# AnyLoc/AnyLoc

Hardware: NVIDIA H100
Metric: images/sec end-to-end DINOv2-VLAD descriptors (higher is better)
Workload: dtype f32-equivalent (tensor-core fp16 3-term split, fp32 accumulate)

## Files before the change

anyloc_b200/csrc/attention_tc.cu:

```cuda
#include <stdlib.h>
#include "common.cuh"

namespace anyloc {
namespace atc {

constexpr int BQ = 64, BKV = 64, HD = 64, WARPS = 4, THREADS = WARPS * 32;

template <bool F16, bool BF16 = false> struct Cfg {
  using T = typename std::conditional<BF16, __nv_bfloat16, typename std::conditional<F16, __half, float>::type>::type;
  static constexpr int PITCH = F16 ? HD + 8 : HD + 4;
  static constexpr int MAT = BKV * PITCH;
  static constexpr int NMAT = BF16 ? 2 : 4;
  static constexpr int STAGE = NMAT * MAT;
  static constexpr int SMEM_BYTES = 2 * STAGE * (int)sizeof(T);
  static constexpr int CHUNKS_PER_ROW = HD * (int)sizeof(T) / 16;
};

__device__ __forceinline__ void cp_async16(uint32_t dst, const void* src, bool valid) {
  asm volatile("cp.async.cg.shared.global [%0], [%1], 16, %2;" ::"r"(dst), "l"(src), "r"(valid ? 16 : 0) : "memory");
}
__device__ __forceinline__ void cp_async_commit() { asm volatile("cp.async.commit_group;" ::: "memory"); }
template <int N>
__device__ __forceinline__ void cp_async_wait() { asm volatile("cp.async.wait_group %0;" ::"n"(N) : "memory"); }

__device__ __forceinline__ void mma_f16(float* d, const uint32_t* a, uint32_t b0, uint32_t b1) {
  asm volatile(
      "mma.sync.aligned.m16n8k16.row.col.f32.f16.f16.f32 {%0, %1, %2, %3}, {%4, %5, %6, %7}, {%8, %9}, "
      "{%0, %1, %2, %3};"
      : "+f"(d[0]), "+f"(d[1]), "+f"(d[2]), "+f"(d[3])
      : "r"(a[0]), "r"(a[1]), "r"(a[2]), "r"(a[3]), "r"(b0), "r"(b1));
}
__device__ __forceinline__ void mma_bf16(float* d, const uint32_t* a, uint32_t b0, uint32_t b1) {
  asm volatile(
      "mma.sync.aligned.m16n8k16.row.col.f32.bf16.bf16.f32 {%0, %1, %2, %3}, {%4, %5, %6, %7}, {%8, %9}, "
      "{%0, %1, %2, %3};"
      : "+f"(d[0]), "+f"(d[1]), "+f"(d[2]), "+f"(d[3])
      : "r"(a[0]), "r"(a[1]), "r"(a[2]), "r"(a[3]), "r"(b0), "r"(b1));
}
__device__ __forceinline__ void mma_tf32(float* d, const uint32_t* a, uint32_t b0, uint32_t b1) {
  asm volatile(
      "mma.sync.aligned.m16n8k8.row.col.f32.tf32.tf32.f32 {%0, %1, %2, %3}, {%4, %5, %6, %7}, {%8, %9}, "
      "{%0, %1, %2, %3};"
      : "+f"(d[0]), "+f"(d[1]), "+f"(d[2]), "+f"(d[3])
      : "r"(a[0]), "r"(a[1]), "r"(a[2]), "r"(a[3]), "r"(b0), "r"(b1));
}
__device__ __forceinline__ void ldsm_x4(uint32_t addr, uint32_t* r) {
  asm volatile("ldmatrix.sync.aligned.m8n8.x4.shared.b16 {%0, %1, %2, %3}, [%4];"
               : "=r"(r[0]), "=r"(r[1]), "=r"(r[2]), "=r"(r[3]) : "r"(addr));
}
__device__ __forceinline__ void ldsm_x4_t(uint32_t addr, uint32_t* r) {
  asm volatile("ldmatrix.sync.aligned.m8n8.x4.trans.shared.b16 {%0, %1, %2, %3}, [%4];"
               : "=r"(r[0]), "=r"(r[1]), "=r"(r[2]), "=r"(r[3]) : "r"(addr));
}
__device__ __forceinline__ float ex2(float x) {
  float y; asm("ex2.approx.ftz.f32 %0, %1;" : "=f"(y) : "f"(x)); return y;
}
__device__ __forceinline__ uint32_t f2u(float x) { return __float_as_uint(x); }
template <typename E>
__device__ __forceinline__ uint32_t ld_h2(const E* p) { return *reinterpret_cast<const uint32_t*>(p); }

template <bool F16, bool VARLEN, bool BF16 = false>
__device__ __forceinline__ void attention_cta(const void* __restrict__ qkv_hi_, const void* __restrict__ qkv_lo_, int T,
                                              int D, void* __restrict__ o_hi_, void* __restrict__ o_lo_,
                                              const VarlenAttnTable* tab) {
  static_assert(!BF16 || F16, "bf16 uses the 2-byte (k16) layout");
  using C = Cfg<F16, BF16>;
  using E = typename C::T;
  extern __shared__ __align__(16) uint8_t smem_raw[];
  E* smem = reinterpret_cast<E*>(smem_raw);
  const E* qkv_hi = reinterpret_cast<const E*>(qkv_hi_);
  const E* qkv_lo = reinterpret_cast<const E*>(qkv_lo_);
  int qt = blockIdx.x;
  const int h = blockIdx.y, b = blockIdx.z;
  const int warp = threadIdx.x >> 5, lane = threadIdx.x & 31, g = lane >> 2, t4 = lane & 3;
  const size_t ld = 3 * (size_t)D;
  size_t img0 = (size_t)b * T;
  if constexpr (VARLEN) {
    int lo = 0, hi = tab->n - 1;
    while (lo < hi) {
      const int mid = (lo + hi + 1) >> 1;
      if (tab->tile0[mid] <= qt) lo = mid; else hi = mid - 1;
    }
    qt -= tab->tile0[lo]; T = tab->len[lo]; img0 = (size_t)tab->row0[lo];
  }
  const int nblk = (T + BKV - 1) / BKV;
  constexpr bool SCALED = F16 && !BF16;
  const float P_SCALE = SCALED ? 1024.0f : 1.0f;
  const float kScale = 0.125f * 1.4426950408889634f * (SCALED ? 1.0f / (kActScale * kActScale) : 1.0f);

  auto load_block = [&](int j, int buf) {
    E* st = smem + buf * C::STAGE;
    constexpr int PIECES = C::NMAT * BKV * C::CHUNKS_PER_ROW;
    for (int p = threadIdx.x; p < PIECES; p += THREADS) {
      const int mat = p / (BKV * C::CHUNKS_PER_ROW), r = (p / C::CHUNKS_PER_ROW) % BKV, c = p % C::CHUNKS_PER_ROW;
      const int key = j * BKV + r;
      const bool valid = key < T;
      const E* src = (!BF16 && (mat & 1)) ? qkv_lo : qkv_hi;
      const bool is_k = BF16 ? mat == 0 : mat < 2;
      const size_t col = (size_t)(is_k ? D : 2 * D) + (size_t)h * HD + (size_t)c * (16 / sizeof(E));
      const E* gp = src + (valid ? (img0 + key) * ld + col : 0);
      cp_async16((uint32_t)__cvta_generic_to_shared(st + mat * C::MAT + r * C::PITCH + c * (16 / sizeof(E))), gp, valid);
    }
    cp_async_commit();
  };
  load_block(0, 0);

  const int q0 = qt * BQ + warp * 16 + g, q1 = q0 + 8;
  constexpr int QK_STEPS = F16 ? HD / 16 : HD / 8;
  uint32_t qa_hi[QK_STEPS][4], qa_lo[QK_STEPS][4];
  {
    const size_t r0 = (img0 + q0) * ld + (size_t)h * HD, r1 = (img0 + q1) * ld + (size_t)h * HD;
    const bool v0 = q0 < T, v1 = q1 < T;
#pragma unroll
    for (int ks = 0; ks < QK_STEPS; ++ks) {
      if constexpr (F16) {
        const int c0 = ks * 16 + 2 * t4, c1 = c0 + 8;
        qa_hi[ks][0] = v0 ? ld_h2(qkv_hi + r0 + c0) : 0u; qa_hi[ks][1] = v1 ? ld_h2(qkv_hi + r1 + c0) : 0u;
        qa_hi[ks][2] = v0 ? ld_h2(qkv_hi + r0 + c1) : 0u; qa_hi[ks][3] = v1 ? ld_h2(qkv_hi + r1 + c1) : 0u;
        if (BF16) continue;
        qa_lo[ks][0] = v0 ? ld_h2(qkv_lo + r0 + c0) : 0u; qa_lo[ks][1] = v1 ? ld_h2(qkv_lo + r1 + c0) : 0u;
        qa_lo[ks][2] = v0 ? ld_h2(qkv_lo + r0 + c1) : 0u; qa_lo[ks][3] = v1 ? ld_h2(qkv_lo + r1 + c1) : 0u;
      } else {
        const int c0 = ks * 8 + t4, c1 = c0 + 4;
        qa_hi[ks][0] = v0 ? f2u(qkv_hi[r0 + c0]) : 0u; qa_hi[ks][1] = v1 ? f2u(qkv_hi[r1 + c0]) : 0u;
        qa_hi[ks][2] = v0 ? f2u(qkv_hi[r0 + c1]) : 0u; qa_hi[ks][3] = v1 ? f2u(qkv_hi[r1 + c1]) : 0u;
        qa_lo[ks][0] = v0 ? f2u(qkv_lo[r0 + c0]) : 0u; qa_lo[ks][1] = v1 ? f2u(qkv_lo[r1 + c0]) : 0u;
        qa_lo[ks][2] = v0 ? f2u(qkv_lo[r0 + c1]) : 0u; qa_lo[ks][3] = v1 ? f2u(qkv_lo[r1 + c1]) : 0u;
      }
    }
  }

  float o[8][4];
  float m0 = -INFINITY, m1 = -INFINITY, l0 = 0.f, l1 = 0.f;
#pragma unroll
  for (int nd = 0; nd < 8; ++nd) o[nd][0] = o[nd][1] = o[nd][2] = o[nd][3] = 0.f;

  for (int j = 0; j < nblk; ++j) {
    const int buf = j & 1;
    if (j + 1 < nblk) { load_block(j + 1, buf ^ 1); cp_async_wait<1>(); }
    else cp_async_wait<0>();
    __syncthreads();
    const E* sK_hi = smem + buf * C::STAGE;
    const E* sK_lo = sK_hi + C::MAT;
    const E* sV_hi = sK_hi + (BF16 ? 1 : 2) * C::MAT;
    const E* sV_lo = sK_hi + 3 * C::MAT;

    float s[8][4];
#pragma unroll
    for (int nt = 0; nt < 8; ++nt) s[nt][0] = s[nt][1] = s[nt][2] = s[nt][3] = 0.f;
#pragma unroll
    for (int nt = 0; nt < 8; ++nt) {
      if constexpr (F16) {
        const int key = nt * 8 + (lane & 7), dim = 8 * (lane >> 3);
#pragma unroll
        for (int c = 0; c < 2; ++c) {
          uint32_t bh[4], bl[4];
          ldsm_x4((uint32_t)__cvta_generic_to_shared(sK_hi + key * C::PITCH + 32 * c + dim), bh);
          if constexpr (BF16) {
#pragma unroll
            for (int u = 0; u < 2; ++u) mma_bf16(s[nt], qa_hi[2 * c + u], bh[2 * u], bh[2 * u + 1]);
            continue;
          }
          ldsm_x4((uint32_t)__cvta_generic_to_shared(sK_lo + key * C::PITCH + 32 * c + dim), bl);
#pragma unroll
          for (int u = 0; u < 2; ++u) {
            const int ks = 2 * c + u;
            mma_f16(s[nt], qa_hi[ks], bh[2 * u], bh[2 * u + 1]);
            mma_f16(s[nt], qa_lo[ks], bh[2 * u], bh[2 * u + 1]);
            mma_f16(s[nt], qa_hi[ks], bl[2 * u], bl[2 * u + 1]);
          }
        }
      } else {
        const float* kh = sK_hi + (nt * 8 + g) * C::PITCH;
        const float* kl = sK_lo + (nt * 8 + g) * C::PITCH;
#pragma unroll
        for (int ks = 0; ks < QK_STEPS; ++ks) {
          const uint32_t bh0 = f2u(kh[ks * 8 + t4]), bh1 = f2u(kh[ks * 8 + t4 + 4]);
          const uint32_t bl0 = f2u(kl[ks * 8 + t4]), bl1 = f2u(kl[ks * 8 + t4 + 4]);
          mma_tf32(s[nt], qa_hi[ks], bh0, bh1);
          mma_tf32(s[nt], qa_lo[ks], bh0, bh1);
          mma_tf32(s[nt], qa_hi[ks], bl0, bl1);
        }
      }
    }

    float mx0 = m0, mx1 = m1;
#pragma unroll
    for (int nt = 0; nt < 8; ++nt) {
      const int key = j * BKV + nt * 8 + 2 * t4;
#pragma unroll
      for (int e = 0; e < 2; ++e) {
        const bool live = key + e < T;
        s[nt][e] = live ? s[nt][e] * kScale : -INFINITY;
        s[nt][2 + e] = live ? s[nt][2 + e] * kScale : -INFINITY;
        mx0 = fmaxf(mx0, s[nt][e]); mx1 = fmaxf(mx1, s[nt][2 + e]);
      }
    }
    mx0 = fmaxf(mx0, __shfl_xor_sync(0xffffffffu, mx0, 1)); mx0 = fmaxf(mx0, __shfl_xor_sync(0xffffffffu, mx0, 2));
    mx1 = fmaxf(mx1, __shfl_xor_sync(0xffffffffu, mx1, 1)); mx1 = fmaxf(mx1, __shfl_xor_sync(0xffffffffu, mx1, 2));
    const float alpha0 = ex2(m0 - mx0), alpha1 = ex2(m1 - mx1);
    m0 = mx0; m1 = mx1;
    float r0 = 0.f, r1 = 0.f;
#pragma unroll
    for (int nt = 0; nt < 8; ++nt) {
      s[nt][0] = ex2(s[nt][0] - mx0); s[nt][1] = ex2(s[nt][1] - mx0);
      s[nt][2] = ex2(s[nt][2] - mx1); s[nt][3] = ex2(s[nt][3] - mx1);
      r0 += s[nt][0] + s[nt][1]; r1 += s[nt][2] + s[nt][3];
    }
    l0 = l0 * alpha0 + r0; l1 = l1 * alpha1 + r1;

    float pv[8][4];
#pragma unroll
    for (int nd = 0; nd < 8; ++nd) pv[nd][0] = pv[nd][1] = pv[nd][2] = pv[nd][3] = 0.f;
    if constexpr (BF16) {
#pragma unroll
      for (int ks = 0; ks < 4; ++ks) {
        uint32_t ph[4];
        ph[0] = pack_bf16x2(s[2 * ks][0], s[2 * ks][1]);
        ph[1] = pack_bf16x2(s[2 * ks][2], s[2 * ks][3]);
        ph[2] = pack_bf16x2(s[2 * ks + 1][0], s[2 * ks + 1][1]);
        ph[3] = pack_bf16x2(s[2 * ks + 1][2], s[2 * ks + 1][3]);
        const int key = ks * 16 + (lane & 7) + 8 * ((lane >> 3) & 1), dsel = 8 * (lane >> 4);
#pragma unroll
        for (int nd = 0; nd < 8; nd += 2) {
          uint32_t vh[4];
          ldsm_x4_t((uint32_t)__cvta_generic_to_shared(sV_hi + key * C::PITCH + nd * 8 + dsel), vh);
#pragma unroll
          for (int u = 0; u < 2; ++u) mma_bf16(pv[nd + u], ph, vh[2 * u], vh[2 * u + 1]);
        }
      }
    } else if constexpr (F16) {
#pragma unroll
      for (int ks = 0; ks < 4; ++ks) {
        uint32_t ph[4], pl[4];
        split_f16x2(s[2 * ks][0] * P_SCALE, s[2 * ks][1] * P_SCALE, ph[0], pl[0]);
        split_f16x2(s[2 * ks][2] * P_SCALE, s[2 * ks][3] * P_SCALE, ph[1], pl[1]);
        split_f16x2(s[2 * ks + 1][0] * P_SCALE, s[2 * ks + 1][1] * P_SCALE, ph[2], pl[2]);
        split_f16x2(s[2 * ks + 1][2] * P_SCALE, s[2 * ks + 1][3] * P_SCALE, ph[3], pl[3]);
        const int key = ks * 16 + (lane & 7) + 8 * ((lane >> 3) & 1), dsel = 8 * (lane >> 4);
#pragma unroll
        for (int nd = 0; nd < 8; nd += 2) {
          uint32_t vh[4], vl[4];
          ldsm_x4_t((uint32_t)__cvta_generic_to_shared(sV_hi + key * C::PITCH + nd * 8 + dsel), vh);
          ldsm_x4_t((uint32_t)__cvta_generic_to_shared(sV_lo + key * C::PITCH + nd * 8 + dsel), vl);
#pragma unroll
          for (int u = 0; u < 2; ++u) {
            mma_f16(pv[nd + u], ph, vh[2 * u], vh[2 * u + 1]);
            mma_f16(pv[nd + u], pl, vh[2 * u], vh[2 * u + 1]);
            mma_f16(pv[nd + u], ph, vl[2 * u], vl[2 * u + 1]);
          }
        }
      }
    } else {
#pragma unroll
      for (int ks = 0; ks < 8; ++ks) {
        uint32_t ph[4], pl[4];
        float hh, ll;
        split_tf32(s[ks][0], hh, ll); ph[0] = f2u(hh); pl[0] = f2u(ll);
        split_tf32(s[ks][2], hh, ll); ph[1] = f2u(hh); pl[1] = f2u(ll);
        split_tf32(s[ks][1], hh, ll); ph[2] = f2u(hh); pl[2] = f2u(ll);
        split_tf32(s[ks][3], hh, ll); ph[3] = f2u(hh); pl[3] = f2u(ll);
        const float* vh0 = sV_hi + (ks * 8 + 2 * t4) * C::PITCH;
        const float* vl0 = sV_lo + (ks * 8 + 2 * t4) * C::PITCH;
#pragma unroll
        for (int nd = 0; nd < 8; ++nd) {
          const uint32_t bh0 = f2u(vh0[nd * 8 + g]), bh1 = f2u(vh0[C::PITCH + nd * 8 + g]);
          const uint32_t bl0 = f2u(vl0[nd * 8 + g]), bl1 = f2u(vl0[C::PITCH + nd * 8 + g]);
          mma_tf32(pv[nd], ph, bh0, bh1);
          mma_tf32(pv[nd], pl, bh0, bh1);
          mma_tf32(pv[nd], ph, bl0, bl1);
        }
      }
    }
#pragma unroll
    for (int nd = 0; nd < 8; ++nd) {
      o[nd][0] = o[nd][0] * alpha0 + pv[nd][0]; o[nd][1] = o[nd][1] * alpha0 + pv[nd][1];
      o[nd][2] = o[nd][2] * alpha1 + pv[nd][2]; o[nd][3] = o[nd][3] * alpha1 + pv[nd][3];
    }
    __syncthreads();
  }

  l0 += __shfl_xor_sync(0xffffffffu, l0, 1); l0 += __shfl_xor_sync(0xffffffffu, l0, 2);
  l1 += __shfl_xor_sync(0xffffffffu, l1, 1); l1 += __shfl_xor_sync(0xffffffffu, l1, 2);
  const float inv0 = 1.0f / (l0 * P_SCALE), inv1 = 1.0f / (l1 * P_SCALE);
#pragma unroll
  for (int half = 0; half < 2; ++half) {
    const int q = half ? q1 : q0;
    if (q >= T) continue;
    const float inv = half ? inv1 : inv0;
    const size_t off = (img0 + q) * (size_t)D + (size_t)h * HD + 2 * t4;
#pragma unroll
    for (int nd = 0; nd < 8; ++nd) {
      const float a = o[nd][2 * half] * inv, c = o[nd][2 * half + 1] * inv;
      if constexpr (BF16) {
        *reinterpret_cast<uint32_t*>(reinterpret_cast<__nv_bfloat16*>(o_hi_) + off + nd * 8) = pack_bf16x2(a, c);
      } else if constexpr (F16) {
        uint32_t hh, ll;
        split_f16x2(a, c, hh, ll);
        *reinterpret_cast<uint32_t*>(reinterpret_cast<__half*>(o_hi_) + off + nd * 8) = hh;
        *reinterpret_cast<uint32_t*>(reinterpret_cast<__half*>(o_lo_) + off + nd * 8) = ll;
      } else {
        float2 hh, ll;
        split_tf32(a, hh.x, ll.x); split_tf32(c, hh.y, ll.y);
        *reinterpret_cast<float2*>(reinterpret_cast<float*>(o_hi_) + off + nd * 8) = hh;
        *reinterpret_cast<float2*>(reinterpret_cast<float*>(o_lo_) + off + nd * 8) = ll;
      }
    }
  }
}

template <bool F16, bool BF16 = false>
__global__ void __launch_bounds__(THREADS)
attention_tc_kernel(const void* __restrict__ qkv_hi_, const void* __restrict__ qkv_lo_, int T, int D,
                    void* __restrict__ o_hi_, void* __restrict__ o_lo_) {
  attention_cta<F16, false, BF16>(qkv_hi_, qkv_lo_, T, D, o_hi_, o_lo_, nullptr);
}

template <bool F16, bool BF16 = false>
__global__ void __launch_bounds__(THREADS)
attention_tc_varlen_kernel(const void* __restrict__ qkv_hi_, const void* __restrict__ qkv_lo_,
                           const __grid_constant__ VarlenAttnTable tab, int D, void* __restrict__ o_hi_,
                           void* __restrict__ o_lo_) {
  attention_cta<F16, true, BF16>(qkv_hi_, qkv_lo_, 0, D, o_hi_, o_lo_, &tab);
}

__global__ void __launch_bounds__(256)
qkv_to_f16_kernel(const float* __restrict__ qkv_hi, const float* __restrict__ qkv_lo, size_t n, __half* __restrict__ q16_hi,
                  __half* __restrict__ q16_lo) {
  for (size_t i = blockIdx.x * (size_t)blockDim.x + threadIdx.x; i < n; i += (size_t)gridDim.x * blockDim.x) {
    __half hh, ll; split_f16((qkv_hi[i] + qkv_lo[i]) * kActScale, hh, ll);
    q16_hi[i] = hh; q16_lo[i] = ll;
  }
}

}

int attention_tc_launch(const void* qkv_hi, const void* qkv_lo, int B, int T, int D, int heads, void* o_hi, void* o_lo,
                        int fmt, cudaStream_t st) {
  using namespace atc;
  ANYLOC_REQUIRE(D == heads * HD, "attention_tc: head_dim must be 64 (D=%d heads=%d)", D, heads);
  ANYLOC_REQUIRE(B <= 65535 && heads <= 65535, "attention_tc: grid too large (B=%d heads=%d)", B, heads);
  static unsigned long long attr_seen = 0;
  if (first_use_on_this_device(&attr_seen)) {
    ANYLOC_CHECK_CUDA(cudaFuncSetAttribute(attention_tc_kernel<true>, cudaFuncAttributeMaxDynamicSharedMemorySize,
                                           Cfg<true>::SMEM_BYTES));
    ANYLOC_CHECK_CUDA(cudaFuncSetAttribute(attention_tc_kernel<false>, cudaFuncAttributeMaxDynamicSharedMemorySize,
                                           Cfg<false>::SMEM_BYTES));
  }
  const dim3 grid(cdiv(T, BQ), heads, B);
  if (fmt == ANYLOC_PAIR_BF16)
    attention_tc_kernel<true, true><<<grid, THREADS, Cfg<true, true>::SMEM_BYTES, st>>>(qkv_hi, qkv_lo, T, D, o_hi, o_lo);
  else if (fmt == ANYLOC_PAIR_F16) attention_tc_kernel<true><<<grid, THREADS, Cfg<true>::SMEM_BYTES, st>>>(qkv_hi, qkv_lo, T, D, o_hi, o_lo);
  else attention_tc_kernel<false><<<grid, THREADS, Cfg<false>::SMEM_BYTES, st>>>(qkv_hi, qkv_lo, T, D, o_hi, o_lo);
  ANYLOC_CHECK_LAUNCH();
  return ANYLOC_OK;
}

int attention_tc_varlen_launch(const void* qkv_hi, const void* qkv_lo, const VarlenAttnTable& tab, int n_tiles, int D,
                               int heads, void* o_hi, void* o_lo, int fmt, cudaStream_t st) {
  using namespace atc;
  ANYLOC_REQUIRE(D == heads * HD, "attention_tc: head_dim must be 64 (D=%d heads=%d)", D, heads);
  ANYLOC_REQUIRE(heads <= 65535, "attention_tc: grid too large (heads=%d)", heads);
  static unsigned long long attr_seen = 0;
  if (first_use_on_this_device(&attr_seen)) {
    ANYLOC_CHECK_CUDA(cudaFuncSetAttribute(attention_tc_varlen_kernel<true>,
                                           cudaFuncAttributeMaxDynamicSharedMemorySize, Cfg<true>::SMEM_BYTES));
    ANYLOC_CHECK_CUDA(cudaFuncSetAttribute(attention_tc_varlen_kernel<false>,
                                           cudaFuncAttributeMaxDynamicSharedMemorySize, Cfg<false>::SMEM_BYTES));
  }
  const dim3 grid(n_tiles, heads);
  if (fmt == ANYLOC_PAIR_BF16)
    attention_tc_varlen_kernel<true, true><<<grid, THREADS, Cfg<true, true>::SMEM_BYTES, st>>>(qkv_hi, qkv_lo, tab, D,
                                                                                             o_hi, o_lo);
  else if (fmt == ANYLOC_PAIR_F16)
    attention_tc_varlen_kernel<true><<<grid, THREADS, Cfg<true>::SMEM_BYTES, st>>>(qkv_hi, qkv_lo, tab, D, o_hi, o_lo);
  else
    attention_tc_varlen_kernel<false><<<grid, THREADS, Cfg<false>::SMEM_BYTES, st>>>(qkv_hi, qkv_lo, tab, D, o_hi, o_lo);
  ANYLOC_CHECK_LAUNCH();
  return ANYLOC_OK;
}

int attention_tc16_standalone(const float* qkv_hi, const float* qkv_lo, int B, int T, int D, int heads, void* o_hi,
                              void* o_lo, cudaStream_t st) {
  const size_t nq = (size_t)B * T * 3 * D;
  __half* buf = nullptr;
  ANYLOC_CHECK_CUDA(cudaMallocAsync((void**)&buf, 2 * nq * sizeof(__half), st));
  const int blocks = (int)std::min<size_t>((nq + 255) / 256, (size_t)device_sm_count() * 16);
  atc::qkv_to_f16_kernel<<<blocks, 256, 0, st>>>(qkv_hi, qkv_lo, nq, buf, buf + nq);
  ANYLOC_CHECK_LAUNCH();
  int rc = attention_tc_launch(buf, buf + nq, B, T, D, heads, o_hi, o_lo, ANYLOC_PAIR_F16, st);
  cudaFreeAsync(buf, st);
  return rc;
}

}
```

anyloc_b200/csrc/gemm_tc.cu:

```cuda
#include <cuda.h>
#include <stdlib.h>
#include "epilogue.cuh"
#include "tc_common.cuh"

namespace anyloc {

namespace tc {

constexpr int BM = 128, BN = 128;
constexpr int KSTEPS = 4;
constexpr int A_BYTES = BM * 128;
constexpr int B_BYTES = BN * 128;
constexpr int THREADS = 384;
constexpr int STG_BYTES = 8192;

template <bool LO, bool STG = LO> struct Cfg {
  static constexpr int STAGE_BYTES = (LO ? 2 : 1) * (A_BYTES + B_BYTES);
  static constexpr int B_OFF = (LO ? 2 : 1) * A_BYTES;
  static constexpr int STAGES = LO ? 3 : 6;
  static constexpr int BAR_OFF = STAGES * STAGE_BYTES;
  static constexpr int SMEM_BYTES = BAR_OFF + 256 + 1024 ;
  static constexpr bool STAGED = STG;
  static constexpr int STG_OFF = BAR_OFF + 1024;
  static constexpr int SMEM_BYTES_STAGED = STG_OFF + 4 * STG_BYTES + 1024 ;
};
constexpr int BAND_N = 16;
constexpr int CHUNK_KB_TF32 = 2;
constexpr int CHUNK_KB_F16 = 8;
constexpr int CHUNK_KB_COARSE = 32;

__device__ __forceinline__ void tile_coords(int tile, int num_m, int num_n, int band_n, int& m_blk, int& n_blk) {
  const int per_band = num_m * band_n;
  const int band = tile / per_band, r = tile - band * per_band;
  const int w = min(band_n, num_n - band * band_n);
  m_blk = r / w;
  n_blk = band * band_n + (r - m_blk * w);
}

template <bool BF16 = false>
__device__ __forceinline__ void store_split2(const EpiParams& ep, size_t o, float a, float b) {
  if (BF16) {
    *reinterpret_cast<uint32_t*>(reinterpret_cast<__nv_bfloat16*>(ep.out) + o) = pack_bf16x2(a, b);
  } else if (ep.out_f16) {
    uint32_t h, l;
    split_f16x2(a * kActScale, b * kActScale, h, l);
    *reinterpret_cast<uint32_t*>(reinterpret_cast<__half*>(ep.out) + o) = h;
    *reinterpret_cast<uint32_t*>(reinterpret_cast<__half*>(ep.out_lo) + o) = l;
  } else {
    float2 h, l;
    split_tf32(a, h.x, l.x); split_tf32(b, h.y, l.y);
    *reinterpret_cast<float2*>(ep.out + o) = h;
    *reinterpret_cast<float2*>(ep.out_lo + o) = l;
  }
}

template <bool BF16 = false>
__device__ __forceinline__ void epi_pair(const EpiParams& ep, int m, int n, int N, float v0, float v1) {
  const int mode = ep.mode;
  if (mode < 0) return;
  if (mode == ANYLOC_EPI_SWIGLU_SPLIT) {
    epi_store_pair<BF16>(ep, m, n, v0, v1);
    return;
  }
  if (n + 1 >= N || (ep.ldo & 1)) {
    epi_store1<BF16>(ep, m, n, v0);
    if (n + 1 < N) epi_store1<BF16>(ep, m, n + 1, v1);
    return;
  }
  const float al = ep.alpha;
  float2 b = make_float2(0.f, 0.f);
  if (ep.bias) b = __ldg(reinterpret_cast<const float2*>(ep.bias + n));
  const float x0 = v0 * al + b.x, x1 = v1 * al + b.y;
  const size_t o = (size_t)m * ep.ldo + n;
  if (mode == ANYLOC_EPI_BIAS) {
    *reinterpret_cast<float2*>(ep.out + o) = make_float2(x0, x1);
  } else if (mode == ANYLOC_EPI_LS_RESID) {
    const float2 g = __ldg(reinterpret_cast<const float2*>(ep.gamma + n));
    const float2 r = *reinterpret_cast<const float2*>(ep.resid + o);
    *reinterpret_cast<float2*>(ep.out + o) = make_float2(r.x + g.x * x0, r.y + g.y * x1);
  } else if (mode == ANYLOC_EPI_GELU_SPLIT) {
    store_split2<BF16>(ep, o, gelu_erf(x0), gelu_erf(x1));
  } else {
    store_split2<BF16>(ep, o, x0, x1);
  }
}

template <bool BF16 = false>
__device__ __forceinline__ void epilogue_pairs(const EpiParams& ep, int r0, int nq, int M, int N, const float* sum) {
#pragma unroll
  for (int j = 0; j < 16; ++j) {
    const int n = nq + j * 8;
    if (n >= N) continue;
    if (r0 < M) epi_pair<BF16>(ep, r0, n, N, sum[4 * j], sum[4 * j + 1]);
    if (r0 + 8 < M) epi_pair<BF16>(ep, r0 + 8, n, N, sum[4 * j + 2], sum[4 * j + 3]);
  }
}

__device__ __forceinline__ void epilogue_regs_batched(const EpiParams& ep, int r0, int nq, int M, int N, const float* sum) {
  const int mode = ep.mode;
  if (mode < 0) return;
  const int n0 = nq & ~(BN - 1);
  const bool swiglu = mode == ANYLOC_EPI_SWIGLU_SPLIT, resid = mode == ANYLOC_EPI_LS_RESID;
  if (n0 + BN > N || (!swiglu && (ep.ldo & 1))) {
    epilogue_pairs(ep, r0, nq, M, N, sum);
    return;
  }
  const bool row0 = r0 < M, row1 = r0 + 8 < M;
  const size_t o0 = (size_t)r0 * ep.ldo, o1 = (size_t)(r0 + 8) * ep.ldo;
  const float al = ep.alpha;
#pragma unroll
  for (int j0 = 0; j0 < 16; j0 += 2) {
    float2 b[2], g[2], ra[2], rb[2];
#pragma unroll
    for (int jj = 0; jj < 2; ++jj) {
      const int n = nq + (j0 + jj) * 8;
      b[jj] = ep.bias ? __ldg(reinterpret_cast<const float2*>(ep.bias + n)) : make_float2(0.f, 0.f);
      if (resid) {
        g[jj] = __ldg(reinterpret_cast<const float2*>(ep.gamma + n));
        if (row0) ra[jj] = *reinterpret_cast<const float2*>(ep.resid + o0 + n);
        if (row1) rb[jj] = *reinterpret_cast<const float2*>(ep.resid + o1 + n);
      }
    }
#pragma unroll
    for (int jj = 0; jj < 2; ++jj) {
      const int j = j0 + jj, n = nq + j * 8;
#pragma unroll
      for (int h = 0; h < 2; ++h) {
        if (!(h ? row1 : row0)) continue;
        const float v0 = sum[4 * j + 2 * h], v1 = sum[4 * j + 2 * h + 1];
        const size_t ro = h ? o1 : o0;
        if (swiglu) {
          const float x1 = v0 * al + b[jj].x, x2 = v1 * al + b[jj].y;
          epi_store_split(ep, ro + (n >> 1), silu(x1) * x2);
          continue;
        }
        const float x0 = v0 * al + b[jj].x, x1 = v1 * al + b[jj].y;
        const size_t o = ro + n;
        if (mode == ANYLOC_EPI_BIAS) {
          *reinterpret_cast<float2*>(ep.out + o) = make_float2(x0, x1);
        } else if (resid) {
          const float2 r = h ? rb[jj] : ra[jj];
          *reinterpret_cast<float2*>(ep.out + o) = make_float2(r.x + g[jj].x * x0, r.y + g[jj].y * x1);
        } else if (mode == ANYLOC_EPI_GELU_SPLIT) {
          store_split2(ep, o, gelu_erf(x0), gelu_erf(x1));
        } else {
          store_split2(ep, o, x0, x1);
        }
      }
    }
  }
}

enum StageKind { STG_F32 = 0, STG_F16_PAIR = 1, STG_TF32_PAIR = 2, STG_BF16 = 3 };
constexpr int STG_HALF = STG_BYTES / 2;
constexpr int STG_ROWS = 64;

template <int KIND>
struct StageFmt {
  static constexpr int ESZ = KIND == STG_F16_PAIR || KIND == STG_BF16 ? 2 : 4;
  static constexpr int COLS = KIND == STG_TF32_PAIR ? 16 : KIND == STG_BF16 ? 64 : 32;
  static constexpr int ROW_BYTES = COLS * ESZ;
  static constexpr uint32_t SWZ = ROW_BYTES == 128 ? 7 : 3;
};

template <int KIND>
__device__ __forceinline__ uint32_t stg_off(int row, int b) {
  const uint32_t o = (uint32_t)(row * StageFmt<KIND>::ROW_BYTES + b);
  return o ^ (((o >> 7) & StageFmt<KIND>::SWZ) << 4);
}

__device__ __forceinline__ float2 ldg_col_pair(const float* p, int n, int N) {
  if (n + 1 < N) return __ldg(reinterpret_cast<const float2*>(p + n));
  return make_float2(n < N ? __ldg(p + n) : 0.f, 0.f);
}

__device__ __forceinline__ void resid_load(const CUtensorMap* tm, uint8_t* buf, uint64_t* bar, int oc, int m0) {
  mbar_expect_tx(smem_u32(bar), STG_BYTES);
  tma_load_2d(smem_u32(buf), tm, smem_u32(bar), oc, m0);
}

template <int KIND, bool SWIGLU, bool RESID>
__device__ __forceinline__ void epilogue_staged(const EpiParams& ep, const CUtensorMap* tm_out, const CUtensorMap* tm_lo,
                                                const CUtensorMap* tm_resid, uint8_t* stg, uint64_t* rbar,
                                                uint32_t& rphase, uint32_t& cnt, int wg, int t, int m0, int n0, int N,
                                                const float* sum) {
  using F = StageFmt<KIND>;
  constexpr int ACC = SWIGLU ? 2 * F::COLS : F::COLS;
  constexpr int JS = ACC / 8;
  const int lane = t & 31, q = lane & 3, row = (t >> 5) * 16 + (lane >> 2);
  const int n_out = SWIGLU ? N >> 1 : N;
  const int oc_base = SWIGLU ? n0 >> 1 : n0;
  const bool gelu = ep.mode == ANYLOC_EPI_GELU_SPLIT;
  const float al = ep.alpha;
#pragma unroll
  for (int s = 0; s < BN / ACC; ++s) {
    const int oc0 = oc_base + s * F::COLS;
    if (oc0 >= n_out) break;
    const uint32_t b = cnt & 1;
    uint8_t* buf = stg + b * STG_BYTES;
    if (RESID) { mbar_wait(smem_u32(rbar + b), (rphase >> b) & 1); rphase ^= 1u << b; }
#pragma unroll
    for (int jj = 0; jj < JS; ++jj) {
      const int j = s * JS + jj, n = n0 + j * 8 + 2 * q;
      const float2 bb = ep.bias ? ldg_col_pair(ep.bias, n, N) : make_float2(0.f, 0.f);
      float2 g;
      if (RESID) g = ldg_col_pair(ep.gamma, n, N);
#pragma unroll
      for (int h = 0; h < 2; ++h) {
        const int r = row + 8 * h;
        const float x0 = sum[4 * j + 2 * h] * al + bb.x, x1 = sum[4 * j + 2 * h + 1] * al + bb.y;
        if (SWIGLU) {
          const float v = silu(x0) * x1;
          const uint32_t o = stg_off<KIND>(r, (4 * jj + q) * F::ESZ);
          if (KIND == STG_BF16) {
            *reinterpret_cast<__nv_bfloat16*>(buf + o) = __float2bfloat16_rn(v);
          } else if (KIND == STG_F16_PAIR) {
            __half hi, lo;
            split_f16(v * kActScale, hi, lo);
            *reinterpret_cast<__half*>(buf + o) = hi;
            *reinterpret_cast<__half*>(buf + STG_HALF + o) = lo;
          } else {
            float hi, lo;
            split_tf32(v, hi, lo);
            *reinterpret_cast<float*>(buf + o) = hi;
            *reinterpret_cast<float*>(buf + STG_HALF + o) = lo;
          }
          continue;
        }
        const uint32_t o = stg_off<KIND>(r, (8 * jj + 2 * q) * F::ESZ);
        if (KIND == STG_F32) {
          float2* p = reinterpret_cast<float2*>(buf + o);
          if (RESID) {
            const float2 rr = *p;
            *p = make_float2(rr.x + g.x * x0, rr.y + g.y * x1);
          } else {
            *p = make_float2(x0, x1);
          }
        } else {
          const float y0 = gelu ? gelu_erf(x0) : x0, y1 = gelu ? gelu_erf(x1) : x1;
          if (KIND == STG_BF16) {
            *reinterpret_cast<uint32_t*>(buf + o) = pack_bf16x2(y0, y1);
          } else if (KIND == STG_F16_PAIR) {
            uint32_t hi, lo;
            split_f16x2(y0 * kActScale, y1 * kActScale, hi, lo);
            *reinterpret_cast<uint32_t*>(buf + o) = hi;
            *reinterpret_cast<uint32_t*>(buf + STG_HALF + o) = lo;
          } else {
            float2 hi, lo;
            split_tf32(y0, hi.x, lo.x); split_tf32(y1, hi.y, lo.y);
            *reinterpret_cast<float2*>(buf + o) = hi;
            *reinterpret_cast<float2*>(buf + STG_HALF + o) = lo;
          }
        }
      }
    }
    fence_proxy_async_smem();
    if (t == 0) bulk_wait_read<0>();
    if (wg == 1) named_bar_sync<1>(128);
    else named_bar_sync<2>(128);
    if (t == 0) {
      tma_store_2d(tm_out, smem_u32(buf), oc0, m0);
      if (KIND != STG_F32 && KIND != STG_BF16) tma_store_2d(tm_lo, smem_u32(buf + STG_HALF), oc0, m0);
      bulk_commit();
      if (RESID && s + 2 < BN / ACC && oc0 + 2 * F::COLS < n_out) {
        bulk_wait_read<0>();
        resid_load(tm_resid, buf, rbar + b, oc0 + 2 * F::COLS, m0);
      }
    }
    ++cnt;
  }
}

template <bool F16, int LOM, bool BF16 = false>
__global__ void __launch_bounds__(THREADS, 1)
gemm_tc3_kernel(const __grid_constant__ CUtensorMap tm_a_hi, const __grid_constant__ CUtensorMap tm_a_lo,
                const __grid_constant__ CUtensorMap tm_b_hi, const __grid_constant__ CUtensorMap tm_b_lo,
                const __grid_constant__ CUtensorMap tm_out, const __grid_constant__ CUtensorMap tm_out_lo,
                const __grid_constant__ CUtensorMap tm_resid, int staged,
                int M, int N, int K, int band_n, int chunk_kb, EpiParams ep) {
  constexpr bool LO = LOM != 0, has_a_lo = (LOM & 1) != 0, has_b_lo = (LOM & 2) != 0;
  static_assert(!BF16 || (F16 && LOM == 0), "bf16 is a single-operand 2-byte format");
  using C = Cfg<LO, LO || BF16>;
  if (ep.gate != nullptr && *reinterpret_cast<const volatile int*>(ep.gate) == 0) return;
  extern __shared__ uint8_t smem_raw[];
  uint8_t* smem = reinterpret_cast<uint8_t*>((reinterpret_cast<uintptr_t>(smem_raw) + 1023) & ~(uintptr_t)1023);
  uint64_t* full_bar = reinterpret_cast<uint64_t*>(smem + C::BAR_OFF);
  uint64_t* empty_bar = full_bar + C::STAGES;
  uint64_t* resid_bar = empty_bar + C::STAGES;

  const int wg = threadIdx.x >> 7;
  const int num_m = (M + BM - 1) / BM, num_n = (N + BN - 1) / BN;
  const int num_tiles = num_m * num_n;
  constexpr int BKE = F16 ? 64 : 32;
  const int num_k = (K + BKE - 1) / BKE;

  if (threadIdx.x == 0) {
    asm volatile("prefetch.tensormap [%0];" ::"l"(&tm_a_hi) : "memory");
    asm volatile("prefetch.tensormap [%0];" ::"l"(&tm_b_hi) : "memory");
    for (int s = 0; s < C::STAGES; ++s) { mbar_init(smem_u32(full_bar + s), 1); mbar_init(smem_u32(empty_bar + s), 2); }
    if (C::STAGED)
      for (int i = 0; i < 4; ++i) mbar_init(smem_u32(resid_bar + i), 1);
    asm volatile("fence.mbarrier_init.release.cluster;" ::: "memory");
  }
  __syncthreads();

  if (wg == 0) {
    if (threadIdx.x == 0) {
      const uint32_t tx_bytes = A_BYTES * (1 + ((LO && has_a_lo) ? 1 : 0)) + B_BYTES * (1 + ((LO && has_b_lo) ? 1 : 0));
      int stage = 0; uint32_t phase = 0;
      for (int tile = blockIdx.x; tile < num_tiles; tile += gridDim.x) {
        int mb, nb; tile_coords(tile, num_m, num_n, band_n, mb, nb);
        const int m0 = mb * BM, n0 = nb * BN;
        for (int kb = 0; kb < num_k; ++kb) {
          mbar_wait(smem_u32(empty_bar + stage), phase ^ 1);
          const uint32_t fb = smem_u32(full_bar + stage);
          mbar_expect_tx(fb, tx_bytes);
          const uint32_t sbase = smem_u32(smem + stage * C::STAGE_BYTES);
          tma_load_2d(sbase, &tm_a_hi, fb, kb * BKE, m0);
          if (LO && has_a_lo) tma_load_2d(sbase + A_BYTES, &tm_a_lo, fb, kb * BKE, m0);
          tma_load_2d(sbase + C::B_OFF, &tm_b_hi, fb, kb * BKE, n0);
          if (LO && has_b_lo) tma_load_2d(sbase + C::B_OFF + B_BYTES, &tm_b_lo, fb, kb * BKE, n0);
          if (++stage == C::STAGES) { stage = 0; phase ^= 1; }
        }
      }
    }
    return;
  }

  const int t = threadIdx.x & 127, warp = t >> 5, lane = t & 31;
  const uint32_t a_sub = (uint32_t)(wg - 1) * 64 * 128;
  uint8_t* stg = smem + C::STG_OFF + (wg - 1) * 2 * STG_BYTES;
  uint64_t* rbar = resid_bar + (wg - 1) * 2;
  const int mode = ep.mode;
  staged = C::STAGED && staged;
  const bool resid_staged = staged && mode == ANYLOC_EPI_LS_RESID;
  uint32_t stg_cnt = 0, rphase = 0;
  int stage = 0; uint32_t phase = 0;
  for (int tile = blockIdx.x; tile < num_tiles; tile += gridDim.x) {
    int mb, nb; tile_coords(tile, num_m, num_n, band_n, mb, nb);
    const int m0 = mb * BM + (wg - 1) * 64, n0 = nb * BN;
    float sum[64], acc[64];
#pragma unroll
    for (int j = 0; j < 64; ++j) { sum[j] = 0.f; acc[j] = 0.f; }
    int prev_stage = -1;
    for (int kb0 = 0; kb0 < num_k; kb0 += chunk_kb) {
      const int kb1 = min(num_k, kb0 + chunk_kb);
      if (resid_staged && kb1 == num_k && t == 0 && m0 < M) {
        bulk_wait_read<0>();
        for (int i = 0; i < 2; ++i) {
          const uint32_t b = (stg_cnt + i) & 1;
          const int oc = n0 + i * StageFmt<STG_F32>::COLS;
          if (oc < N) resid_load(&tm_resid, stg + b * STG_BYTES, rbar + b, oc, m0);
        }
      }
      for (int kb = kb0; kb < kb1; ++kb) {
        mbar_wait(smem_u32(full_bar + stage), phase);
        const uint32_t sbase = smem_u32(smem + stage * C::STAGE_BYTES);
        const uint64_t a_hi = make_desc(sbase + a_sub), a_lo = make_desc(sbase + A_BYTES + a_sub);
        const uint64_t b_hi = make_desc(sbase + C::B_OFF), b_lo = make_desc(sbase + C::B_OFF + B_BYTES);
        wgmma_fence();
#pragma unroll
        for (int k = 0; k < KSTEPS; ++k) {
          const uint64_t adv = (uint64_t)((k * 32) >> 4);
          if constexpr (BF16) wgmma_m64n128_bf16(acc, a_hi + adv, b_hi + adv, (kb != kb0 || k != 0) ? 1u : 0u);
          else wgmma_m64n128<F16>(acc, a_hi + adv, b_hi + adv, (kb != kb0 || k != 0) ? 1u : 0u);
          if (has_a_lo) wgmma_m64n128<F16>(acc, a_lo + adv, b_hi + adv, 1u);
          if (has_b_lo) wgmma_m64n128<F16>(acc, a_hi + adv, b_lo + adv, 1u);
        }
        wgmma_commit();
        wgmma_wait<1>();
        if (prev_stage >= 0 && t == 0) mbar_arrive(smem_u32(empty_bar + prev_stage));
        prev_stage = stage;
        if (++stage == C::STAGES) { stage = 0; phase ^= 1; }
      }
      wgmma_wait<0>();
      fence_regs<64>(acc);
#pragma unroll
      for (int j = 0; j < 64; ++j) sum[j] += acc[j];
    }
    if (t == 0) mbar_arrive(smem_u32(empty_bar + prev_stage));
    if (mode < 0 || m0 >= M) continue;
    if constexpr (!C::STAGED) {
      epilogue_regs_batched(ep, m0 + warp * 16 + (lane >> 2), n0 + 2 * (lane & 3), M, N, sum);
      continue;
    }
    if (!staged) {
      epilogue_pairs<BF16>(ep, m0 + warp * 16 + (lane >> 2), n0 + 2 * (lane & 3), M, N, sum);
      continue;
    }
#define ANYLOC_EPI_STAGED(KIND_, SWIGLU_, RESID_)                                                                   \
  epilogue_staged<KIND_, SWIGLU_, RESID_>(ep, &tm_out, &tm_out_lo, &tm_resid, stg, rbar, rphase, stg_cnt, wg, t, m0, \
                                          n0, N, sum)
    if (mode == ANYLOC_EPI_BIAS) ANYLOC_EPI_STAGED(STG_F32, false, false);
    else if (mode == ANYLOC_EPI_LS_RESID) ANYLOC_EPI_STAGED(STG_F32, false, true);
    else if (BF16) {
      if (mode == ANYLOC_EPI_SWIGLU_SPLIT) ANYLOC_EPI_STAGED(STG_BF16, true, false);
      else ANYLOC_EPI_STAGED(STG_BF16, false, false);
    } else if (mode == ANYLOC_EPI_SWIGLU_SPLIT) {
      if (ep.out_f16) ANYLOC_EPI_STAGED(STG_F16_PAIR, true, false);
      else ANYLOC_EPI_STAGED(STG_TF32_PAIR, true, false);
    } else {
      if (ep.out_f16) ANYLOC_EPI_STAGED(STG_F16_PAIR, false, false);
      else ANYLOC_EPI_STAGED(STG_TF32_PAIR, false, false);
    }
#undef ANYLOC_EPI_STAGED
  }
  if (staged && t == 0) bulk_wait<0>();
}

typedef CUresult (*EncodeTiledFn)(CUtensorMap*, CUtensorMapDataType, cuuint32_t, void*, const cuuint64_t*,
                                  const cuuint64_t*, const cuuint32_t*, const cuuint32_t*, CUtensorMapInterleave,
                                  CUtensorMapSwizzle, CUtensorMapL2promotion, CUtensorMapFloatOOBfill);

static EncodeTiledFn get_encode() {
  static EncodeTiledFn fn = nullptr;
  if (!fn) {
    void* p = nullptr;
    cudaDriverEntryPointQueryResult q;
    if (cudaGetDriverEntryPoint("cuTensorMapEncodeTiled", &p, cudaEnableDefault, &q) != cudaSuccess ||
        q != cudaDriverEntryPointSuccess)
      return nullptr;
    fn = (EncodeTiledFn)p;
  }
  return fn;
}

int make_map(CUtensorMap* map, const void* ptr, int rows, int K, int ld, int box_rows, bool f16, bool bf16) {
  EncodeTiledFn enc = get_encode();
  if (!enc) { set_error("gemm_tc: cuTensorMapEncodeTiled unavailable"); return ANYLOC_ERR_CUDA; }
  const int esz = f16 ? 2 : 4;
  cuuint64_t dims[2] = {(cuuint64_t)K, (cuuint64_t)rows};
  cuuint64_t strides[1] = {(cuuint64_t)ld * esz};
  cuuint32_t box[2] = {(cuuint32_t)(128 / esz), (cuuint32_t)box_rows};
  cuuint32_t estr[2] = {1, 1};
  const CUtensorMapDataType dt = bf16 ? CU_TENSOR_MAP_DATA_TYPE_BFLOAT16
                                 : f16 ? CU_TENSOR_MAP_DATA_TYPE_FLOAT16 : CU_TENSOR_MAP_DATA_TYPE_FLOAT32;
  CUresult r = enc(map, dt, 2, (void*)ptr, dims, strides, box, estr, CU_TENSOR_MAP_INTERLEAVE_NONE, CU_TENSOR_MAP_SWIZZLE_128B,
                   CU_TENSOR_MAP_L2_PROMOTION_L2_256B, CU_TENSOR_MAP_FLOAT_OOB_FILL_NONE);
  if (r != CUDA_SUCCESS) { set_error("gemm_tc: cuTensorMapEncodeTiled failed (%d) rows=%d K=%d ld=%d", (int)r, rows, K, ld); return ANYLOC_ERR_CUDA; }
  return ANYLOC_OK;
}

static int make_out_map(CUtensorMap* map, const void* ptr, int rows, int cols, int ld, int esz, int box_cols,
                        bool bf16 = false) {
  EncodeTiledFn enc = get_encode();
  if (!enc) { set_error("gemm_tc: cuTensorMapEncodeTiled unavailable"); return ANYLOC_ERR_CUDA; }
  cuuint64_t dims[2] = {(cuuint64_t)cols, (cuuint64_t)rows};
  cuuint64_t strides[1] = {(cuuint64_t)ld * esz};
  cuuint32_t box[2] = {(cuuint32_t)box_cols, (cuuint32_t)STG_ROWS};
  cuuint32_t estr[2] = {1, 1};
  const CUtensorMapDataType dt = bf16 ? CU_TENSOR_MAP_DATA_TYPE_BFLOAT16
                                 : esz == 2 ? CU_TENSOR_MAP_DATA_TYPE_FLOAT16 : CU_TENSOR_MAP_DATA_TYPE_FLOAT32;
  CUresult r = enc(map, dt, 2, (void*)ptr, dims, strides, box, estr, CU_TENSOR_MAP_INTERLEAVE_NONE,
                   box_cols * esz == 128 ? CU_TENSOR_MAP_SWIZZLE_128B : CU_TENSOR_MAP_SWIZZLE_64B,
                   CU_TENSOR_MAP_L2_PROMOTION_L2_256B, CU_TENSOR_MAP_FLOAT_OOB_FILL_NONE);
  if (r != CUDA_SUCCESS) { set_error("gemm_tc: cuTensorMapEncodeTiled failed (%d) for the output: rows=%d cols=%d ld=%d", (int)r, rows, cols, ld); return ANYLOC_ERR_CUDA; }
  return ANYLOC_OK;
}

static int make_epi_maps(const EpiParams& ep, int M, int N, CUtensorMap* m_out, CUtensorMap* m_lo, CUtensorMap* m_resid,
                         bool* staged, bool bf16) {
  memset(m_out, 0, sizeof(*m_out)); memset(m_lo, 0, sizeof(*m_lo)); memset(m_resid, 0, sizeof(*m_resid));
  const bool split = ep.mode == ANYLOC_EPI_BIAS_SPLIT || ep.mode == ANYLOC_EPI_GELU_SPLIT ||
                     ep.mode == ANYLOC_EPI_SWIGLU_SPLIT;
  const int esz = split && (ep.out_f16 || bf16) ? 2 : 4;
  const int n_out = ep.mode == ANYLOC_EPI_SWIGLU_SPLIT ? N / 2 : N;
  *staged = ep.mode >= 0 && ((long long)ep.ldo * esz) % 16 == 0 && ((long long)n_out * esz) % 16 == 0;
  if (!*staged) return ANYLOC_OK;
  const int cols = split && bf16 ? StageFmt<STG_BF16>::COLS
                   : split && !ep.out_f16 ? StageFmt<STG_TF32_PAIR>::COLS : StageFmt<STG_F32>::COLS;
  int rc;
  if ((rc = make_out_map(m_out, ep.out, M, n_out, ep.ldo, esz, cols, split && bf16))) return rc;
  if (split && !bf16 && (rc = make_out_map(m_lo, ep.out_lo, M, n_out, ep.ldo, esz, cols))) return rc;
  if (ep.mode == ANYLOC_EPI_LS_RESID && (rc = make_out_map(m_resid, ep.resid, M, n_out, ep.ldo, esz, cols))) return rc;
  return ANYLOC_OK;
}

}

bool gemm_tc_supported(const void* a_hi, const void* a_lo, int lda, const void* b_hi, const void* b_lo, int ldb,
                       int M, int N, int K, const EpiParams& ep, bool f16) {
  auto al16 = [](const void* p) { return (reinterpret_cast<uintptr_t>(p) & 15) == 0; };
  const int q = f16 ? 8 : 4;
  if (M < 1 || N < 1 || K < q) return false;
  if ((K % q) || (lda % q) || (ldb % q)) return false;
  if (!al16(a_hi) || !al16(b_hi) || (a_lo && !al16(a_lo)) || (b_lo && !al16(b_lo))) return false;
  if (!al16(ep.out) || (ep.out_lo && !al16(ep.out_lo)) || (ep.resid && !al16(ep.resid))) return false;
  if (ep.bias && !al16(ep.bias)) return false;
  if (ep.gamma && !al16(ep.gamma)) return false;
  return true;
}

static thread_local int g_last_staged = -1;

template <bool F16, int LOM, bool BF16 = false>
static int launch_impl(const void* a_hi, const void* a_lo, int lda, const void* b_hi, const void* b_lo, int ldb, int M,
                       int N, int K, const EpiParams& ep, int chunk, cudaStream_t st) {
  using namespace tc;
  constexpr bool LO = LOM != 0;
  using CF = Cfg<LO, LO || BF16>;
  CUtensorMap ma_hi, ma_lo, mb_hi, mb_lo;
  int rc;
  if ((rc = make_map(&ma_hi, a_hi, M, K, lda, BM, F16, BF16))) return rc;
  if ((rc = make_map(&ma_lo, a_lo ? a_lo : a_hi, M, K, lda, BM, F16, BF16))) return rc;
  if ((rc = make_map(&mb_hi, b_hi, N, K, ldb, BN, F16, BF16))) return rc;
  if ((rc = make_map(&mb_lo, b_lo ? b_lo : b_hi, N, K, ldb, BN, F16, BF16))) return rc;
  CUtensorMap mo, mo_lo, mr;
  bool staged = false;
  memset(&mo, 0, sizeof(mo)); memset(&mo_lo, 0, sizeof(mo_lo)); memset(&mr, 0, sizeof(mr));
  if (CF::STAGED && ep.gate == nullptr && (rc = make_epi_maps(ep, M, N, &mo, &mo_lo, &mr, &staged, BF16))) return rc;
  const int smem = staged ? CF::SMEM_BYTES_STAGED : CF::SMEM_BYTES;
  g_last_staged = staged ? 1 : 0;
  static unsigned long long attr_seen = 0;
  if (first_use_on_this_device(&attr_seen)) {
    ANYLOC_CHECK_CUDA(cudaFuncSetAttribute(gemm_tc3_kernel<F16, LOM, BF16>, cudaFuncAttributeMaxDynamicSharedMemorySize,
                                           CF::STAGED ? CF::SMEM_BYTES_STAGED : CF::SMEM_BYTES));
  }
  const int tiles = cdiv(M, BM) * cdiv(N, BN);
  const int grid = std::min(tiles, device_sm_count());
  gemm_tc3_kernel<F16, LOM, BF16><<<grid, THREADS, smem, st>>>(
      ma_hi, ma_lo, mb_hi, mb_lo, mo, mo_lo, mr, staged ? 1 : 0, M, N, K, std::min(BAND_N, cdiv(N, BN)), chunk, ep);
  ANYLOC_CHECK_LAUNCH();
  return ANYLOC_OK;
}

int gemm_tc_launch(const void* a_hi, const void* a_lo, int lda, const void* b_hi, const void* b_lo, int ldb, int M,
                   int N, int K, const EpiParams& ep_in, bool f16, cudaStream_t st) {
  static int chunk_env = -1;
  if (chunk_env < 0) { const char* e = getenv("ANYLOC_GEMM_CHUNK"); chunk_env = e ? atoi(e) : 0; }
  static int skip_epi = -1;
  if (skip_epi < 0) { const char* e = getenv("ANYLOC_GEMM_DEBUG_SKIP_EPI"); skip_epi = e ? atoi(e) : 0; }
  EpiParams ep = ep_in;
  if (skip_epi && ((skip_epi >> ep_in.mode) & 1)) ep.mode = -1;
  const int lom = (a_lo ? 1 : 0) | (b_lo ? 2 : 0);
  const int chunk = lom == 0 ? (f16 ? tc::CHUNK_KB_COARSE : tc::CHUNK_KB_TF32)
                             : chunk_env > 0 ? chunk_env : (f16 ? tc::CHUNK_KB_F16 : tc::CHUNK_KB_TF32);
#define ANYLOC_GEMM_LAUNCH(F16_, LOM_) launch_impl<F16_, LOM_>(a_hi, a_lo, lda, b_hi, b_lo, ldb, M, N, K, ep, chunk, st)
  switch (lom + (f16 ? 4 : 0)) {
    case 0: return ANYLOC_GEMM_LAUNCH(false, 0);
    case 1: return ANYLOC_GEMM_LAUNCH(false, 1);
    case 2: return ANYLOC_GEMM_LAUNCH(false, 2);
    case 3: return ANYLOC_GEMM_LAUNCH(false, 3);
    case 4: return ANYLOC_GEMM_LAUNCH(true, 0);
    case 5: return ANYLOC_GEMM_LAUNCH(true, 1);
    case 6: return ANYLOC_GEMM_LAUNCH(true, 2);
    default: return ANYLOC_GEMM_LAUNCH(true, 3);
  }
#undef ANYLOC_GEMM_LAUNCH
}

int gemm_tc_bf16_launch(const void* a, int lda, const void* b, int ldb, int M, int N, int K, const EpiParams& ep,
                        cudaStream_t st) {
  static_assert(tc::Cfg<false, true>::SMEM_BYTES_STAGED <= 232448, "bf16 GEMM over H100's shared-memory opt-in");
  return launch_impl<true, 0, true>(a, nullptr, lda, b, nullptr, ldb, M, N, K, ep, tc::CHUNK_KB_F16, st);
}

}

extern "C" int anyloc_gemm_tc_last_staged(void) { return anyloc::g_last_staged; }
```

anyloc_b200/csrc/tc_common.cuh:

```cuda
#pragma once
#include <cuda.h>
#include "common.cuh"

namespace anyloc {
namespace tc {

__device__ __forceinline__ uint32_t smem_u32(const void* p) { return (uint32_t)__cvta_generic_to_shared(p); }

__device__ __forceinline__ void mbar_init(uint32_t bar, uint32_t count) {
  asm volatile("mbarrier.init.shared::cta.b64 [%0], %1;" ::"r"(bar), "r"(count));
}
__device__ __forceinline__ void mbar_expect_tx(uint32_t bar, uint32_t bytes) {
  asm volatile("mbarrier.arrive.expect_tx.shared::cta.b64 _, [%0], %1;" ::"r"(bar), "r"(bytes) : "memory");
}
__device__ __forceinline__ void mbar_arrive(uint32_t bar) {
  asm volatile("mbarrier.arrive.shared::cta.b64 _, [%0];" ::"r"(bar) : "memory");
}
__device__ __forceinline__ void mbar_wait(uint32_t bar, uint32_t parity) {
  uint32_t done = 0;
  long long t0 = 0;
  for (uint32_t it = 0; !done; ++it) {
    asm volatile(
        "{\n\t.reg .pred p;\n\t"
        "mbarrier.try_wait.parity.shared::cta.b64 p, [%1], %2;\n\t"
        "selp.u32 %0, 1, 0, p;\n\t}"
        : "=r"(done) : "r"(bar), "r"(parity) : "memory");
    if (!done && (it & 0x3ff) == 0x3ff) {
      long long now = clock64();
      if (t0 == 0) t0 = now;
      else if (now - t0 > 8000000000LL) __trap();
    }
  }
}
__device__ __forceinline__ void tma_load_2d(uint32_t dst, const CUtensorMap* map, uint32_t bar, int c0, int c1) {
  asm volatile(
      "cp.async.bulk.tensor.2d.shared::cluster.global.mbarrier::complete_tx::bytes [%0], [%1, {%3, %4}], [%2];"
      ::"r"(dst), "l"(map), "r"(bar), "r"(c0), "r"(c1) : "memory");
}

__device__ __forceinline__ void tma_store_2d(const CUtensorMap* map, uint32_t src, int c0, int c1) {
  asm volatile("cp.async.bulk.tensor.2d.global.shared::cta.bulk_group [%0, {%2, %3}], [%1];"
               ::"l"(map), "r"(src), "r"(c0), "r"(c1) : "memory");
}
__device__ __forceinline__ void bulk_commit() { asm volatile("cp.async.bulk.commit_group;" ::: "memory"); }
template <int N>
__device__ __forceinline__ void bulk_wait_read() { asm volatile("cp.async.bulk.wait_group.read %0;" ::"n"(N) : "memory"); }
template <int N>
__device__ __forceinline__ void bulk_wait() { asm volatile("cp.async.bulk.wait_group %0;" ::"n"(N) : "memory"); }
__device__ __forceinline__ void fence_proxy_async_smem() { asm volatile("fence.proxy.async.shared::cta;" ::: "memory"); }
template <int ID>
__device__ __forceinline__ void named_bar_sync(int count) {
  asm volatile("bar.sync %0, %1;" ::"n"(ID), "r"(count) : "memory");
}

__device__ __forceinline__ uint64_t make_desc(uint32_t saddr) {
  uint64_t d = 0;
  d |= (uint64_t)((saddr & 0x3FFFF) >> 4);
  d |= (uint64_t)1 << 16;
  d |= (uint64_t)(1024 >> 4) << 32;
  d |= (uint64_t)1 << 62;
  return d;
}

__device__ __forceinline__ void wgmma_fence() { asm volatile("wgmma.fence.sync.aligned;" ::: "memory"); }
__device__ __forceinline__ void wgmma_commit() { asm volatile("wgmma.commit_group.sync.aligned;" ::: "memory"); }
template <int N>
__device__ __forceinline__ void wgmma_wait() { asm volatile("wgmma.wait_group.sync.aligned %0;" ::"n"(N) : "memory"); }
template <int R>
__device__ __forceinline__ void fence_regs(float* d) {
#pragma unroll
  for (int i = 0; i < R; ++i) asm volatile("" : "+f"(d[i])::"memory");
}

template <bool F16>
__device__ __forceinline__ void wgmma_m64n128(float* d, uint64_t adesc, uint64_t bdesc, uint32_t scale_d) {
  if constexpr (F16)
    asm volatile(
        "{\n\t.reg .pred p;\n\tsetp.ne.b32 p, %66, 0;\n\t"
        "wgmma.mma_async.sync.aligned.m64n128k16.f32.f16.f16 "
        "{%0, %1, %2, %3, %4, %5, %6, %7, %8, %9, %10, %11, %12, %13, %14, %15, %16, %17, %18, %19, %20, %21, %22, "
        "%23, %24, %25, %26, %27, %28, %29, %30, %31, %32, %33, %34, %35, %36, %37, %38, %39, %40, %41, %42, %43, %44, "
        "%45, %46, %47, %48, %49, %50, %51, %52, %53, %54, %55, %56, %57, %58, %59, %60, %61, %62, %63}, "
        "%64, %65, p, 1, 1, 0, 0;\n\t}"
        : "+f"(d[0]), "+f"(d[1]), "+f"(d[2]), "+f"(d[3]), "+f"(d[4]), "+f"(d[5]), "+f"(d[6]), "+f"(d[7]),
          "+f"(d[8]), "+f"(d[9]), "+f"(d[10]), "+f"(d[11]), "+f"(d[12]), "+f"(d[13]), "+f"(d[14]), "+f"(d[15]),
          "+f"(d[16]), "+f"(d[17]), "+f"(d[18]), "+f"(d[19]), "+f"(d[20]), "+f"(d[21]), "+f"(d[22]), "+f"(d[23]),
          "+f"(d[24]), "+f"(d[25]), "+f"(d[26]), "+f"(d[27]), "+f"(d[28]), "+f"(d[29]), "+f"(d[30]), "+f"(d[31]),
          "+f"(d[32]), "+f"(d[33]), "+f"(d[34]), "+f"(d[35]), "+f"(d[36]), "+f"(d[37]), "+f"(d[38]), "+f"(d[39]),
          "+f"(d[40]), "+f"(d[41]), "+f"(d[42]), "+f"(d[43]), "+f"(d[44]), "+f"(d[45]), "+f"(d[46]), "+f"(d[47]),
          "+f"(d[48]), "+f"(d[49]), "+f"(d[50]), "+f"(d[51]), "+f"(d[52]), "+f"(d[53]), "+f"(d[54]), "+f"(d[55]),
          "+f"(d[56]), "+f"(d[57]), "+f"(d[58]), "+f"(d[59]), "+f"(d[60]), "+f"(d[61]), "+f"(d[62]), "+f"(d[63])
        : "l"(adesc), "l"(bdesc), "r"(scale_d));
  else
    asm volatile(
        "{\n\t.reg .pred p;\n\tsetp.ne.b32 p, %66, 0;\n\t"
        "wgmma.mma_async.sync.aligned.m64n128k8.f32.tf32.tf32 "
        "{%0, %1, %2, %3, %4, %5, %6, %7, %8, %9, %10, %11, %12, %13, %14, %15, %16, %17, %18, %19, %20, %21, %22, "
        "%23, %24, %25, %26, %27, %28, %29, %30, %31, %32, %33, %34, %35, %36, %37, %38, %39, %40, %41, %42, %43, %44, "
        "%45, %46, %47, %48, %49, %50, %51, %52, %53, %54, %55, %56, %57, %58, %59, %60, %61, %62, %63}, "
        "%64, %65, p, 1, 1;\n\t}"
        : "+f"(d[0]), "+f"(d[1]), "+f"(d[2]), "+f"(d[3]), "+f"(d[4]), "+f"(d[5]), "+f"(d[6]), "+f"(d[7]),
          "+f"(d[8]), "+f"(d[9]), "+f"(d[10]), "+f"(d[11]), "+f"(d[12]), "+f"(d[13]), "+f"(d[14]), "+f"(d[15]),
          "+f"(d[16]), "+f"(d[17]), "+f"(d[18]), "+f"(d[19]), "+f"(d[20]), "+f"(d[21]), "+f"(d[22]), "+f"(d[23]),
          "+f"(d[24]), "+f"(d[25]), "+f"(d[26]), "+f"(d[27]), "+f"(d[28]), "+f"(d[29]), "+f"(d[30]), "+f"(d[31]),
          "+f"(d[32]), "+f"(d[33]), "+f"(d[34]), "+f"(d[35]), "+f"(d[36]), "+f"(d[37]), "+f"(d[38]), "+f"(d[39]),
          "+f"(d[40]), "+f"(d[41]), "+f"(d[42]), "+f"(d[43]), "+f"(d[44]), "+f"(d[45]), "+f"(d[46]), "+f"(d[47]),
          "+f"(d[48]), "+f"(d[49]), "+f"(d[50]), "+f"(d[51]), "+f"(d[52]), "+f"(d[53]), "+f"(d[54]), "+f"(d[55]),
          "+f"(d[56]), "+f"(d[57]), "+f"(d[58]), "+f"(d[59]), "+f"(d[60]), "+f"(d[61]), "+f"(d[62]), "+f"(d[63])
        : "l"(adesc), "l"(bdesc), "r"(scale_d));
}

__device__ __forceinline__ void wgmma_m64n128_bf16(float* d, uint64_t adesc, uint64_t bdesc, uint32_t scale_d) {
  asm volatile(
      "{\n\t.reg .pred p;\n\tsetp.ne.b32 p, %66, 0;\n\t"
      "wgmma.mma_async.sync.aligned.m64n128k16.f32.bf16.bf16 "
      "{%0, %1, %2, %3, %4, %5, %6, %7, %8, %9, %10, %11, %12, %13, %14, %15, %16, %17, %18, %19, %20, %21, %22, "
      "%23, %24, %25, %26, %27, %28, %29, %30, %31, %32, %33, %34, %35, %36, %37, %38, %39, %40, %41, %42, %43, %44, "
      "%45, %46, %47, %48, %49, %50, %51, %52, %53, %54, %55, %56, %57, %58, %59, %60, %61, %62, %63}, "
      "%64, %65, p, 1, 1, 0, 0;\n\t}"
      : "+f"(d[0]), "+f"(d[1]), "+f"(d[2]), "+f"(d[3]), "+f"(d[4]), "+f"(d[5]), "+f"(d[6]), "+f"(d[7]),
        "+f"(d[8]), "+f"(d[9]), "+f"(d[10]), "+f"(d[11]), "+f"(d[12]), "+f"(d[13]), "+f"(d[14]), "+f"(d[15]),
        "+f"(d[16]), "+f"(d[17]), "+f"(d[18]), "+f"(d[19]), "+f"(d[20]), "+f"(d[21]), "+f"(d[22]), "+f"(d[23]),
        "+f"(d[24]), "+f"(d[25]), "+f"(d[26]), "+f"(d[27]), "+f"(d[28]), "+f"(d[29]), "+f"(d[30]), "+f"(d[31]),
        "+f"(d[32]), "+f"(d[33]), "+f"(d[34]), "+f"(d[35]), "+f"(d[36]), "+f"(d[37]), "+f"(d[38]), "+f"(d[39]),
        "+f"(d[40]), "+f"(d[41]), "+f"(d[42]), "+f"(d[43]), "+f"(d[44]), "+f"(d[45]), "+f"(d[46]), "+f"(d[47]),
        "+f"(d[48]), "+f"(d[49]), "+f"(d[50]), "+f"(d[51]), "+f"(d[52]), "+f"(d[53]), "+f"(d[54]), "+f"(d[55]),
        "+f"(d[56]), "+f"(d[57]), "+f"(d[58]), "+f"(d[59]), "+f"(d[60]), "+f"(d[61]), "+f"(d[62]), "+f"(d[63])
      : "l"(adesc), "l"(bdesc), "r"(scale_d));
}

int make_map(CUtensorMap* map, const void* ptr, int rows, int K, int ld, int box_rows, bool f16, bool bf16 = false);

}
}
```

Before: 170.8.

## Route fp16/bf16 attention to a new Hopper wgmma kernel with TMA loads

Adds a new attention kernel for the fp16 and bf16 pair formats. It loads K/V tiles with 3D TMA tensor maps into 128B-swizzled shared memory and computes QK^T and PV with warpgroup wgmma (shared-shared and register-sourced forms), with register reallocation helpers. The old mma.sync kernel is reduced to the tf32 path only. This aims to raise tensor-core throughput and cut load-issue overhead in attention, at the cost of per-call tensor-map encoding on the host and a larger, more complex kernel whose correctness depends on the descriptor and swizzle setup.

```diff
diff --git a/anyloc_b200/csrc/attention_tc.cu b/anyloc_b200/csrc/attention_tc.cu
--- a/anyloc_b200/csrc/attention_tc.cu
+++ b/anyloc_b200/csrc/attention_tc.cu
@@ -6,11 +6,11 @@
 
 constexpr int BQ = 64, BKV = 64, HD = 64, WARPS = 4, THREADS = WARPS * 32;
 
-template <bool F16, bool BF16 = false> struct Cfg {
-  using T = typename std::conditional<BF16, __nv_bfloat16, typename std::conditional<F16, __half, float>::type>::type;
-  static constexpr int PITCH = F16 ? HD + 8 : HD + 4;
+struct Cfg {
+  using T = float;
+  static constexpr int PITCH = HD + 4;
   static constexpr int MAT = BKV * PITCH;
-  static constexpr int NMAT = BF16 ? 2 : 4;
+  static constexpr int NMAT = 4;
   static constexpr int STAGE = NMAT * MAT;
   static constexpr int SMEM_BYTES = 2 * STAGE * (int)sizeof(T);
   static constexpr int CHUNKS_PER_ROW = HD * (int)sizeof(T) / 16;
@@ -23,20 +23,6 @@
 template <int N>
 __device__ __forceinline__ void cp_async_wait() { asm volatile("cp.async.wait_group %0;" ::"n"(N) : "memory"); }
 
-__device__ __forceinline__ void mma_f16(float* d, const uint32_t* a, uint32_t b0, uint32_t b1) {
-  asm volatile(
-      "mma.sync.aligned.m16n8k16.row.col.f32.f16.f16.f32 {%0, %1, %2, %3}, {%4, %5, %6, %7}, {%8, %9}, "
-      "{%0, %1, %2, %3};"
-      : "+f"(d[0]), "+f"(d[1]), "+f"(d[2]), "+f"(d[3])
-      : "r"(a[0]), "r"(a[1]), "r"(a[2]), "r"(a[3]), "r"(b0), "r"(b1));
-}
-__device__ __forceinline__ void mma_bf16(float* d, const uint32_t* a, uint32_t b0, uint32_t b1) {
-  asm volatile(
-      "mma.sync.aligned.m16n8k16.row.col.f32.bf16.bf16.f32 {%0, %1, %2, %3}, {%4, %5, %6, %7}, {%8, %9}, "
-      "{%0, %1, %2, %3};"
-      : "+f"(d[0]), "+f"(d[1]), "+f"(d[2]), "+f"(d[3])
-      : "r"(a[0]), "r"(a[1]), "r"(a[2]), "r"(a[3]), "r"(b0), "r"(b1));
-}
 __device__ __forceinline__ void mma_tf32(float* d, const uint32_t* a, uint32_t b0, uint32_t b1) {
   asm volatile(
       "mma.sync.aligned.m16n8k8.row.col.f32.tf32.tf32.f32 {%0, %1, %2, %3}, {%4, %5, %6, %7}, {%8, %9}, "
@@ -44,27 +30,16 @@
       : "+f"(d[0]), "+f"(d[1]), "+f"(d[2]), "+f"(d[3])
       : "r"(a[0]), "r"(a[1]), "r"(a[2]), "r"(a[3]), "r"(b0), "r"(b1));
 }
-__device__ __forceinline__ void ldsm_x4(uint32_t addr, uint32_t* r) {
-  asm volatile("ldmatrix.sync.aligned.m8n8.x4.shared.b16 {%0, %1, %2, %3}, [%4];"
-               : "=r"(r[0]), "=r"(r[1]), "=r"(r[2]), "=r"(r[3]) : "r"(addr));
-}
-__device__ __forceinline__ void ldsm_x4_t(uint32_t addr, uint32_t* r) {
-  asm volatile("ldmatrix.sync.aligned.m8n8.x4.trans.shared.b16 {%0, %1, %2, %3}, [%4];"
-               : "=r"(r[0]), "=r"(r[1]), "=r"(r[2]), "=r"(r[3]) : "r"(addr));
-}
 __device__ __forceinline__ float ex2(float x) {
   float y; asm("ex2.approx.ftz.f32 %0, %1;" : "=f"(y) : "f"(x)); return y;
 }
 __device__ __forceinline__ uint32_t f2u(float x) { return __float_as_uint(x); }
-template <typename E>
-__device__ __forceinline__ uint32_t ld_h2(const E* p) { return *reinterpret_cast<const uint32_t*>(p); }
-
-template <bool F16, bool VARLEN, bool BF16 = false>
+
+template <bool VARLEN>
 __device__ __forceinline__ void attention_cta(const void* __restrict__ qkv_hi_, const void* __restrict__ qkv_lo_, int T,
                                               int D, void* __restrict__ o_hi_, void* __restrict__ o_lo_,
                                               const VarlenAttnTable* tab) {
-  static_assert(!BF16 || F16, "bf16 uses the 2-byte (k16) layout");
-  using C = Cfg<F16, BF16>;
+  using C = Cfg;
   using E = typename C::T;
   extern __shared__ __align__(16) uint8_t smem_raw[];
   E* smem = reinterpret_cast<E*>(smem_raw);
@@ -84,9 +59,7 @@
     qt -= tab->tile0[lo]; T = tab->len[lo]; img0 = (size_t)tab->row0[lo];
   }
   const int nblk = (T + BKV - 1) / BKV;
-  constexpr bool SCALED = F16 && !BF16;
-  const float P_SCALE = SCALED ? 1024.0f : 1.0f;
-  const float kScale = 0.125f * 1.4426950408889634f * (SCALED ? 1.0f / (kActScale * kActScale) : 1.0f);
+  const float kScale = 0.125f * 1.4426950408889634f;
 
   auto load_block = [&](int j, int buf) {
     E* st = smem + buf * C::STAGE;
@@ -95,8 +68,8 @@
       const int mat = p / (BKV * C::CHUNKS_PER_ROW), r = (p / C::CHUNKS_PER_ROW) % BKV, c = p % C::CHUNKS_PER_ROW;
       const int key = j * BKV + r;
       const bool valid = key < T;
-      const E* src = (!BF16 && (mat & 1)) ? qkv_lo : qkv_hi;
-      const bool is_k = BF16 ? mat == 0 : mat < 2;
+      const E* src = (mat & 1) ? qkv_lo : qkv_hi;
+      const bool is_k = mat < 2;
       const size_t col = (size_t)(is_k ? D : 2 * D) + (size_t)h * HD + (size_t)c * (16 / sizeof(E));
       const E* gp = src + (valid ? (img0 + key) * ld + col : 0);
       cp_async16((uint32_t)__cvta_generic_to_shared(st + mat * C::MAT + r * C::PITCH + c * (16 / sizeof(E))), gp, valid);
@@ -106,27 +79,18 @@
   load_block(0, 0);
 
   const int q0 = qt * BQ + warp * 16 + g, q1 = q0 + 8;
-  constexpr int QK_STEPS = F16 ? HD / 16 : HD / 8;
+  constexpr int QK_STEPS = HD / 8;
   uint32_t qa_hi[QK_STEPS][4], qa_lo[QK_STEPS][4];
   {
     const size_t r0 = (img0 + q0) * ld + (size_t)h * HD, r1 = (img0 + q1) * ld + (size_t)h * HD;
     const bool v0 = q0 < T, v1 = q1 < T;
 #pragma unroll
     for (int ks = 0; ks < QK_STEPS; ++ks) {
-      if constexpr (F16) {
-        const int c0 = ks * 16 + 2 * t4, c1 = c0 + 8;
-        qa_hi[ks][0] = v0 ? ld_h2(qkv_hi + r0 + c0) : 0u; qa_hi[ks][1] = v1 ? ld_h2(qkv_hi + r1 + c0) : 0u;
-        qa_hi[ks][2] = v0 ? ld_h2(qkv_hi + r0 + c1) : 0u; qa_hi[ks][3] = v1 ? ld_h2(qkv_hi + r1 + c1) : 0u;
-        if (BF16) continue;
-        qa_lo[ks][0] = v0 ? ld_h2(qkv_lo + r0 + c0) : 0u; qa_lo[ks][1] = v1 ? ld_h2(qkv_lo + r1 + c0) : 0u;
-        qa_lo[ks][2] = v0 ? ld_h2(qkv_lo + r0 + c1) : 0u; qa_lo[ks][3] = v1 ? ld_h2(qkv_lo + r1 + c1) : 0u;
-      } else {
-        const int c0 = ks * 8 + t4, c1 = c0 + 4;
-        qa_hi[ks][0] = v0 ? f2u(qkv_hi[r0 + c0]) : 0u; qa_hi[ks][1] = v1 ? f2u(qkv_hi[r1 + c0]) : 0u;
-        qa_hi[ks][2] = v0 ? f2u(qkv_hi[r0 + c1]) : 0u; qa_hi[ks][3] = v1 ? f2u(qkv_hi[r1 + c1]) : 0u;
-        qa_lo[ks][0] = v0 ? f2u(qkv_lo[r0 + c0]) : 0u; qa_lo[ks][1] = v1 ? f2u(qkv_lo[r1 + c0]) : 0u;
-        qa_lo[ks][2] = v0 ? f2u(qkv_lo[r0 + c1]) : 0u; qa_lo[ks][3] = v1 ? f2u(qkv_lo[r1 + c1]) : 0u;
-      }
+      const int c0 = ks * 8 + t4, c1 = c0 + 4;
+      qa_hi[ks][0] = v0 ? f2u(qkv_hi[r0 + c0]) : 0u; qa_hi[ks][1] = v1 ? f2u(qkv_hi[r1 + c0]) : 0u;
+      qa_hi[ks][2] = v0 ? f2u(qkv_hi[r0 + c1]) : 0u; qa_hi[ks][3] = v1 ? f2u(qkv_hi[r1 + c1]) : 0u;
+      qa_lo[ks][0] = v0 ? f2u(qkv_lo[r0 + c0]) : 0u; qa_lo[ks][1] = v1 ? f2u(qkv_lo[r1 + c0]) : 0u;
+      qa_lo[ks][2] = v0 ? f2u(qkv_lo[r0 + c1]) : 0u; qa_lo[ks][3] = v1 ? f2u(qkv_lo[r1 + c1]) : 0u;
     }
   }
 
@@ -142,7 +106,7 @@
     __syncthreads();
     const E* sK_hi = smem + buf * C::STAGE;
     const E* sK_lo = sK_hi + C::MAT;
-    const E* sV_hi = sK_hi + (BF16 ? 1 : 2) * C::MAT;
+    const E* sV_hi = sK_hi + 2 * C::MAT;
     const E* sV_lo = sK_hi + 3 * C::MAT;
 
     float s[8][4];
@@ -150,37 +114,15 @@
     for (int nt = 0; nt < 8; ++nt) s[nt][0] = s[nt][1] = s[nt][2] = s[nt][3] = 0.f;
 #pragma unroll
     for (int nt = 0; nt < 8; ++nt) {
-      if constexpr (F16) {
-        const int key = nt * 8 + (lane & 7), dim = 8 * (lane >> 3);
-#pragma unroll
-        for (int c = 0; c < 2; ++c) {
-          uint32_t bh[4], bl[4];
-          ldsm_x4((uint32_t)__cvta_generic_to_shared(sK_hi + key * C::PITCH + 32 * c + dim), bh);
-          if constexpr (BF16) {
-#pragma unroll
-            for (int u = 0; u < 2; ++u) mma_bf16(s[nt], qa_hi[2 * c + u], bh[2 * u], bh[2 * u + 1]);
-            continue;
-          }
-          ldsm_x4((uint32_t)__cvta_generic_to_shared(sK_lo + key * C::PITCH + 32 * c + dim), bl);
-#pragma unroll
-          for (int u = 0; u < 2; ++u) {
-            const int ks = 2 * c + u;
-            mma_f16(s[nt], qa_hi[ks], bh[2 * u], bh[2 * u + 1]);
-            mma_f16(s[nt], qa_lo[ks], bh[2 * u], bh[2 * u + 1]);
-            mma_f16(s[nt], qa_hi[ks], bl[2 * u], bl[2 * u + 1]);
-          }
-        }
-      } else {
-        const float* kh = sK_hi + (nt * 8 + g) * C::PITCH;
-        const float* kl = sK_lo + (nt * 8 + g) * C::PITCH;
-#pragma unroll
-        for (int ks = 0; ks < QK_STEPS; ++ks) {
-          const uint32_t bh0 = f2u(kh[ks * 8 + t4]), bh1 = f2u(kh[ks * 8 + t4 + 4]);
-          const uint32_t bl0 = f2u(kl[ks * 8 + t4]), bl1 = f2u(kl[ks * 8 + t4 + 4]);
-          mma_tf32(s[nt], qa_hi[ks], bh0, bh1);
-          mma_tf32(s[nt], qa_lo[ks], bh0, bh1);
-          mma_tf32(s[nt], qa_hi[ks], bl0, bl1);
-        }
+      const float* kh = sK_hi + (nt * 8 + g) * C::PITCH;
+      const float* kl = sK_lo + (nt * 8 + g) * C::PITCH;
+#pragma unroll
+      for (int ks = 0; ks < QK_STEPS; ++ks) {
+        const uint32_t bh0 = f2u(kh[ks * 8 + t4]), bh1 = f2u(kh[ks * 8 + t4 + 4]);
+        const uint32_t bl0 = f2u(kl[ks * 8 + t4]), bl1 = f2u(kl[ks * 8 + t4 + 4]);
+        mma_tf32(s[nt], qa_hi[ks], bh0, bh1);
+        mma_tf32(s[nt], qa_lo[ks], bh0, bh1);
+        mma_tf32(s[nt], qa_hi[ks], bl0, bl1);
       }
     }
 
@@ -212,64 +154,23 @@
     float pv[8][4];
 #pragma unroll
     for (int nd = 0; nd < 8; ++nd) pv[nd][0] = pv[nd][1] = pv[nd][2] = pv[nd][3] = 0.f;
-    if constexpr (BF16) {
-#pragma unroll
-      for (int ks = 0; ks < 4; ++ks) {
-        uint32_t ph[4];
-        ph[0] = pack_bf16x2(s[2 * ks][0], s[2 * ks][1]);
-        ph[1] = pack_bf16x2(s[2 * ks][2], s[2 * ks][3]);
-        ph[2] = pack_bf16x2(s[2 * ks + 1][0], s[2 * ks + 1][1]);
-        ph[3] = pack_bf16x2(s[2 * ks + 1][2], s[2 * ks + 1][3]);
-        const int key = ks * 16 + (lane & 7) + 8 * ((lane >> 3) & 1), dsel = 8 * (lane >> 4);
-#pragma unroll
-        for (int nd = 0; nd < 8; nd += 2) {
-          uint32_t vh[4];
-          ldsm_x4_t((uint32_t)__cvta_generic_to_shared(sV_hi + key * C::PITCH + nd * 8 + dsel), vh);
-#pragma unroll
-          for (int u = 0; u < 2; ++u) mma_bf16(pv[nd + u], ph, vh[2 * u], vh[2 * u + 1]);
-        }
-      }
-    } else if constexpr (F16) {
-#pragma unroll
-      for (int ks = 0; ks < 4; ++ks) {
-        uint32_t ph[4], pl[4];
-        split_f16x2(s[2 * ks][0] * P_SCALE, s[2 * ks][1] * P_SCALE, ph[0], pl[0]);
-        split_f16x2(s[2 * ks][2] * P_SCALE, s[2 * ks][3] * P_SCALE, ph[1], pl[1]);
-        split_f16x2(s[2 * ks + 1][0] * P_SCALE, s[2 * ks + 1][1] * P_SCALE, ph[2], pl[2]);
-        split_f16x2(s[2 * ks + 1][2] * P_SCALE, s[2 * ks + 1][3] * P_SCALE, ph[3], pl[3]);
-        const int key = ks * 16 + (lane & 7) + 8 * ((lane >> 3) & 1), dsel = 8 * (lane >> 4);
-#pragma unroll
-        for (int nd = 0; nd < 8; nd += 2) {
-          uint32_t vh[4], vl[4];
-          ldsm_x4_t((uint32_t)__cvta_generic_to_shared(sV_hi + key * C::PITCH + nd * 8 + dsel), vh);
-          ldsm_x4_t((uint32_t)__cvta_generic_to_shared(sV_lo + key * C::PITCH + nd * 8 + dsel), vl);
-#pragma unroll
-          for (int u = 0; u < 2; ++u) {
-            mma_f16(pv[nd + u], ph, vh[2 * u], vh[2 * u + 1]);
-            mma_f16(pv[nd + u], pl, vh[2 * u], vh[2 * u + 1]);
-            mma_f16(pv[nd + u], ph, vl[2 * u], vl[2 * u + 1]);
-          }
-        }
-      }
-    } else {
-#pragma unroll
-      for (int ks = 0; ks < 8; ++ks) {
-        uint32_t ph[4], pl[4];
-        float hh, ll;
-        split_tf32(s[ks][0], hh, ll); ph[0] = f2u(hh); pl[0] = f2u(ll);
-        split_tf32(s[ks][2], hh, ll); ph[1] = f2u(hh); pl[1] = f2u(ll);
-        split_tf32(s[ks][1], hh, ll); ph[2] = f2u(hh); pl[2] = f2u(ll);
-        split_tf32(s[ks][3], hh, ll); ph[3] = f2u(hh); pl[3] = f2u(ll);
-        const float* vh0 = sV_hi + (ks * 8 + 2 * t4) * C::PITCH;
-        const float* vl0 = sV_lo + (ks * 8 + 2 * t4) * C::PITCH;
-#pragma unroll
-        for (int nd = 0; nd < 8; ++nd) {
-          const uint32_t bh0 = f2u(vh0[nd * 8 + g]), bh1 = f2u(vh0[C::PITCH + nd * 8 + g]);
-          const uint32_t bl0 = f2u(vl0[nd * 8 + g]), bl1 = f2u(vl0[C::PITCH + nd * 8 + g]);
-          mma_tf32(pv[nd], ph, bh0, bh1);
-          mma_tf32(pv[nd], pl, bh0, bh1);
-          mma_tf32(pv[nd], ph, bl0, bl1);
-        }
+#pragma unroll
+    for (int ks = 0; ks < 8; ++ks) {
+      uint32_t ph[4], pl[4];
+      float hh, ll;
+      split_tf32(s[ks][0], hh, ll); ph[0] = f2u(hh); pl[0] = f2u(ll);
+      split_tf32(s[ks][2], hh, ll); ph[1] = f2u(hh); pl[1] = f2u(ll);
+      split_tf32(s[ks][1], hh, ll); ph[2] = f2u(hh); pl[2] = f2u(ll);
+      split_tf32(s[ks][3], hh, ll); ph[3] = f2u(hh); pl[3] = f2u(ll);
+      const float* vh0 = sV_hi + (ks * 8 + 2 * t4) * C::PITCH;
+      const float* vl0 = sV_lo + (ks * 8 + 2 * t4) * C::PITCH;
+#pragma unroll
+      for (int nd = 0; nd < 8; ++nd) {
+        const uint32_t bh0 = f2u(vh0[nd * 8 + g]), bh1 = f2u(vh0[C::PITCH + nd * 8 + g]);
+        const uint32_t bl0 = f2u(vl0[nd * 8 + g]), bl1 = f2u(vl0[C::PITCH + nd * 8 + g]);
+        mma_tf32(pv[nd], ph, bh0, bh1);
+        mma_tf32(pv[nd], pl, bh0, bh1);
+        mma_tf32(pv[nd], ph, bl0, bl1);
       }
     }
 #pragma unroll
@@ -282,7 +183,7 @@
 
   l0 += __shfl_xor_sync(0xffffffffu, l0, 1); l0 += __shfl_xor_sync(0xffffffffu, l0, 2);
   l1 += __shfl_xor_sync(0xffffffffu, l1, 1); l1 += __shfl_xor_sync(0xffffffffu, l1, 2);
-  const float inv0 = 1.0f / (l0 * P_SCALE), inv1 = 1.0f / (l1 * P_SCALE);
+  const float inv0 = 1.0f / l0, inv1 = 1.0f / l1;
 #pragma unroll
   for (int half = 0; half < 2; ++half) {
     const int q = half ? q1 : q0;
@@ -292,36 +193,25 @@
 #pragma unroll
     for (int nd = 0; nd < 8; ++nd) {
       const float a = o[nd][2 * half] * inv, c = o[nd][2 * half + 1] * inv;
-      if constexpr (BF16) {
-        *reinterpret_cast<uint32_t*>(reinterpret_cast<__nv_bfloat16*>(o_hi_) + off + nd * 8) = pack_bf16x2(a, c);
-      } else if constexpr (F16) {
-        uint32_t hh, ll;
-        split_f16x2(a, c, hh, ll);
-        *reinterpret_cast<uint32_t*>(reinterpret_cast<__half*>(o_hi_) + off + nd * 8) = hh;
-        *reinterpret_cast<uint32_t*>(reinterpret_cast<__half*>(o_lo_) + off + nd * 8) = ll;
-      } else {
-        float2 hh, ll;
-        split_tf32(a, hh.x, ll.x); split_tf32(c, hh.y, ll.y);
-        *reinterpret_cast<float2*>(reinterpret_cast<float*>(o_hi_) + off + nd * 8) = hh;
-        *reinterpret_cast<float2*>(reinterpret_cast<float*>(o_lo_) + off + nd * 8) = ll;
-      }
-    }
-  }
-}
-
-template <bool F16, bool BF16 = false>
+      float2 hh, ll;
+      split_tf32(a, hh.x, ll.x); split_tf32(c, hh.y, ll.y);
+      *reinterpret_cast<float2*>(reinterpret_cast<float*>(o_hi_) + off + nd * 8) = hh;
+      *reinterpret_cast<float2*>(reinterpret_cast<float*>(o_lo_) + off + nd * 8) = ll;
+    }
+  }
+}
+
 __global__ void __launch_bounds__(THREADS)
 attention_tc_kernel(const void* __restrict__ qkv_hi_, const void* __restrict__ qkv_lo_, int T, int D,
                     void* __restrict__ o_hi_, void* __restrict__ o_lo_) {
-  attention_cta<F16, false, BF16>(qkv_hi_, qkv_lo_, T, D, o_hi_, o_lo_, nullptr);
-}
-
-template <bool F16, bool BF16 = false>
+  attention_cta<false>(qkv_hi_, qkv_lo_, T, D, o_hi_, o_lo_, nullptr);
+}
+
 __global__ void __launch_bounds__(THREADS)
 attention_tc_varlen_kernel(const void* __restrict__ qkv_hi_, const void* __restrict__ qkv_lo_,
                            const __grid_constant__ VarlenAttnTable tab, int D, void* __restrict__ o_hi_,
                            void* __restrict__ o_lo_) {
-  attention_cta<F16, true, BF16>(qkv_hi_, qkv_lo_, 0, D, o_hi_, o_lo_, &tab);
+  attention_cta<true>(qkv_hi_, qkv_lo_, 0, D, o_hi_, o_lo_, &tab);
 }
 
 __global__ void __launch_bounds__(256)
@@ -335,23 +225,24 @@
 
 }
 
+int attention_wg_launch(const void* qkv_hi, const void* qkv_lo, int B, int T, int D, int heads, void* o_hi, void* o_lo,
+                        bool bf16, cudaStream_t st);
+int attention_wg_varlen_launch(const void* qkv_hi, const void* qkv_lo, const VarlenAttnTable& tab, int D, int heads,
+                               void* o_hi, void* o_lo, bool bf16, cudaStream_t st);
+
 int attention_tc_launch(const void* qkv_hi, const void* qkv_lo, int B, int T, int D, int heads, void* o_hi, void* o_lo,
                         int fmt, cudaStream_t st) {
   using namespace atc;
   ANYLOC_REQUIRE(D == heads * HD, "attention_tc: head_dim must be 64 (D=%d heads=%d)", D, heads);
   ANYLOC_REQUIRE(B <= 65535 && heads <= 65535, "attention_tc: grid too large (B=%d heads=%d)", B, heads);
+  if (fmt == ANYLOC_PAIR_BF16 || fmt == ANYLOC_PAIR_F16)
+    return attention_wg_launch(qkv_hi, qkv_lo, B, T, D, heads, o_hi, o_lo, fmt == ANYLOC_PAIR_BF16, st);
   static unsigned long long attr_seen = 0;
-  if (first_use_on_this_device(&attr_seen)) {
-    ANYLOC_CHECK_CUDA(cudaFuncSetAttribute(attention_tc_kernel<true>, cudaFuncAttributeMaxDynamicSharedMemorySize,
-                                           Cfg<true>::SMEM_BYTES));
-    ANYLOC_CHECK_CUDA(cudaFuncSetAttribute(attention_tc_kernel<false>, cudaFuncAttributeMaxDynamicSharedMemorySize,
-                                           Cfg<false>::SMEM_BYTES));
-  }
+  if (first_use_on_this_device(&attr_seen))
+    ANYLOC_CHECK_CUDA(cudaFuncSetAttribute(attention_tc_kernel, cudaFuncAttributeMaxDynamicSharedMemorySize,
+                                           Cfg::SMEM_BYTES));
   const dim3 grid(cdiv(T, BQ), heads, B);
-  if (fmt == ANYLOC_PAIR_BF16)
-    attention_tc_kernel<true, true><<<grid, THREADS, Cfg<true, true>::SMEM_BYTES, st>>>(qkv_hi, qkv_lo, T, D, o_hi, o_lo);
-  else if (fmt == ANYLOC_PAIR_F16) attention_tc_kernel<true><<<grid, THREADS, Cfg<true>::SMEM_BYTES, st>>>(qkv_hi, qkv_lo, T, D, o_hi, o_lo);
-  else attention_tc_kernel<false><<<grid, THREADS, Cfg<false>::SMEM_BYTES, st>>>(qkv_hi, qkv_lo, T, D, o_hi, o_lo);
+  attention_tc_kernel<<<grid, THREADS, Cfg::SMEM_BYTES, st>>>(qkv_hi, qkv_lo, T, D, o_hi, o_lo);
   ANYLOC_CHECK_LAUNCH();
   return ANYLOC_OK;
 }
@@ -361,21 +252,14 @@
   using namespace atc;
   ANYLOC_REQUIRE(D == heads * HD, "attention_tc: head_dim must be 64 (D=%d heads=%d)", D, heads);
   ANYLOC_REQUIRE(heads <= 65535, "attention_tc: grid too large (heads=%d)", heads);
+  if (fmt == ANYLOC_PAIR_BF16 || fmt == ANYLOC_PAIR_F16)
+    return attention_wg_varlen_launch(qkv_hi, qkv_lo, tab, D, heads, o_hi, o_lo, fmt == ANYLOC_PAIR_BF16, st);
   static unsigned long long attr_seen = 0;
-  if (first_use_on_this_device(&attr_seen)) {
-    ANYLOC_CHECK_CUDA(cudaFuncSetAttribute(attention_tc_varlen_kernel<true>,
-                                           cudaFuncAttributeMaxDynamicSharedMemorySize, Cfg<true>::SMEM_BYTES));
-    ANYLOC_CHECK_CUDA(cudaFuncSetAttribute(attention_tc_varlen_kernel<false>,
-                                           cudaFuncAttributeMaxDynamicSharedMemorySize, Cfg<false>::SMEM_BYTES));
-  }
+  if (first_use_on_this_device(&attr_seen))
+    ANYLOC_CHECK_CUDA(cudaFuncSetAttribute(attention_tc_varlen_kernel, cudaFuncAttributeMaxDynamicSharedMemorySize,
+                                           Cfg::SMEM_BYTES));
   const dim3 grid(n_tiles, heads);
-  if (fmt == ANYLOC_PAIR_BF16)
-    attention_tc_varlen_kernel<true, true><<<grid, THREADS, Cfg<true, true>::SMEM_BYTES, st>>>(qkv_hi, qkv_lo, tab, D,
-                                                                                             o_hi, o_lo);
-  else if (fmt == ANYLOC_PAIR_F16)
-    attention_tc_varlen_kernel<true><<<grid, THREADS, Cfg<true>::SMEM_BYTES, st>>>(qkv_hi, qkv_lo, tab, D, o_hi, o_lo);
-  else
-    attention_tc_varlen_kernel<false><<<grid, THREADS, Cfg<false>::SMEM_BYTES, st>>>(qkv_hi, qkv_lo, tab, D, o_hi, o_lo);
+  attention_tc_varlen_kernel<<<grid, THREADS, Cfg::SMEM_BYTES, st>>>(qkv_hi, qkv_lo, tab, D, o_hi, o_lo);
   ANYLOC_CHECK_LAUNCH();
   return ANYLOC_OK;
 }
diff --git a/anyloc_b200/csrc/attention_wg.cu b/anyloc_b200/csrc/attention_wg.cu
--- /dev/null
+++ b/anyloc_b200/csrc/attention_wg.cu
@@ -0,0 +1,301 @@
+#include <stdlib.h>
+#include "tc_common.cuh"
+
+namespace anyloc {
+namespace awg {
+
+using namespace tc;
+
+__device__ __forceinline__ float ex2(float x) {
+  float y; asm("ex2.approx.ftz.f32 %0, %1;" : "=f"(y) : "f"(x)); return y;
+}
+
+constexpr int BQ = 128, BKV = 64, HD = 64, THREADS = 384, STAGES = 4;
+constexpr int TILE_BYTES = 64 * 128;
+
+template <bool BF16> struct Cfg {
+  static constexpr int NT = BF16 ? 1 : 2;
+  static constexpr int Q_BYTES = NT * 2 * TILE_BYTES;
+  static constexpr int K_OFF = 0, V_OFF = NT * TILE_BYTES;
+  static constexpr int STAGE_BYTES = 2 * NT * TILE_BYTES;
+  static constexpr int BAR_OFF = Q_BYTES + STAGES * STAGE_BYTES;
+  static constexpr int SMEM_BYTES = BAR_OFF + 256 + 1024 ;
+};
+
+template <bool BF16, bool VARLEN>
+__device__ __forceinline__ void attention_wg_cta(const CUtensorMap* tm_hi, const CUtensorMap* tm_lo, int T, int D,
+                                                 void* __restrict__ o_hi_, void* __restrict__ o_lo_,
+                                                 const VarlenAttnTable* tab) {
+  using C = Cfg<BF16>;
+  extern __shared__ uint8_t smem_raw[];
+  uint8_t* smem = reinterpret_cast<uint8_t*>((reinterpret_cast<uintptr_t>(smem_raw) + 1023) & ~(uintptr_t)1023);
+  uint64_t* full_bar = reinterpret_cast<uint64_t*>(smem + C::BAR_OFF);
+  uint64_t* empty_bar = full_bar + STAGES;
+  uint64_t* q_bar = empty_bar + STAGES;
+
+  int qt = blockIdx.x;
+  const int h = blockIdx.y;
+  int img = blockIdx.z, row0 = 0;
+  size_t out0 = (size_t)blockIdx.z * T;
+  if constexpr (VARLEN) {
+    int lo = 0, hi = tab->n - 1;
+    while (lo < hi) {
+      const int mid = (lo + hi + 1) >> 1;
+      if (tab->tile0[mid] <= qt) lo = mid; else hi = mid - 1;
+    }
+    qt -= tab->tile0[lo]; T = tab->len[lo]; row0 = tab->row0[lo]; img = 0; out0 = (size_t)row0;
+  }
+  const int nblk = (T + BKV - 1) / BKV;
+  const int active = min(2, (T - qt * BQ + 63) / 64);
+  const int wg = threadIdx.x >> 7;
+
+  if (threadIdx.x == 0) {
+    asm volatile("prefetch.tensormap [%0];" ::"l"(tm_hi) : "memory");
+    for (int s = 0; s < STAGES; ++s) { mbar_init(smem_u32(full_bar + s), 1); mbar_init(smem_u32(empty_bar + s), active); }
+    mbar_init(smem_u32(q_bar), 1);
+    asm volatile("fence.mbarrier_init.release.cluster;" ::: "memory");
+  }
+  __syncthreads();
+
+  if (wg == 0) {
+    setmaxnreg_dec<24>();
+    if (threadIdx.x == 0) {
+      const uint32_t qb = smem_u32(q_bar);
+      mbar_expect_tx(qb, C::Q_BYTES);
+      for (int a = 0; a < C::NT; ++a)
+        for (int r = 0; r < 2; ++r)
+          tma_load_3d(smem_u32(smem + (2 * a + r) * TILE_BYTES), a ? tm_lo : tm_hi, qb, h * HD,
+                      row0 + qt * BQ + 64 * r, img);
+      for (int j = 0; j < nblk; ++j) {
+        const int stage = j % STAGES;
+        mbar_wait(smem_u32(empty_bar + stage), ((j / STAGES) & 1) ^ 1);
+        const uint32_t fb = smem_u32(full_bar + stage);
+        mbar_expect_tx(fb, C::STAGE_BYTES);
+        const uint32_t sb = smem_u32(smem + C::Q_BYTES + stage * C::STAGE_BYTES);
+        for (int a = 0; a < C::NT; ++a) {
+          tma_load_3d(sb + C::K_OFF + a * TILE_BYTES, a ? tm_lo : tm_hi, fb, D + h * HD, row0 + j * BKV, img);
+          tma_load_3d(sb + C::V_OFF + a * TILE_BYTES, a ? tm_lo : tm_hi, fb, 2 * D + h * HD, row0 + j * BKV, img);
+        }
+      }
+    }
+    return;
+  }
+
+  setmaxnreg_inc<240>();
+  const int cw = wg - 1;
+  if (qt * BQ + cw * 64 >= T) return;
+  const int t = threadIdx.x & 127, warp = t >> 5, lane = t & 31, g = lane >> 2, t4 = lane & 3;
+  constexpr bool SCALED = !BF16;
+  const float P_SCALE = SCALED ? 1024.0f : 1.0f;
+  const float kScale = 0.125f * 1.4426950408889634f * (SCALED ? 1.0f / (kActScale * kActScale) : 1.0f);
+
+  const uint32_t q_base = smem_u32(smem) + cw * TILE_BYTES;
+  const uint64_t dq_hi = make_desc(q_base), dq_lo = make_desc(q_base + 2 * TILE_BYTES);
+  auto stage_addr = [&](int j) { return smem_u32(smem + C::Q_BYTES + (j % STAGES) * C::STAGE_BYTES); };
+
+  auto issue_s = [&](float* s, int j) {
+    const uint32_t sb = stage_addr(j);
+    const uint64_t dk_hi = make_desc(sb + C::K_OFF), dk_lo = make_desc(sb + C::K_OFF + TILE_BYTES);
+    fence_regs<32>(s);
+    wgmma_fence();
+#pragma unroll
+    for (int k = 0; k < 4; ++k) {
+      const uint64_t adv = (uint64_t)((k * 32) >> 4);
+      wgmma_m64n64_ss<BF16>(s, dq_hi + adv, dk_hi + adv, k != 0 ? 1u : 0u);
+      if constexpr (!BF16) {
+        wgmma_m64n64_ss<false>(s, dq_lo + adv, dk_hi + adv, 1u);
+        wgmma_m64n64_ss<false>(s, dq_hi + adv, dk_lo + adv, 1u);
+      }
+    }
+    wgmma_commit();
+    fence_regs<32>(s);
+  };
+
+  float o[32];
+#pragma unroll
+  for (int i = 0; i < 32; ++i) o[i] = 0.f;
+  float m0 = -INFINITY, m1 = -INFINITY, l0 = 0.f, l1 = 0.f;
+
+  auto block = [&](float* sc, float* sn, int j) {
+    if (j + 1 < nblk) {
+      mbar_wait(smem_u32(full_bar + (j + 1) % STAGES), ((j + 1) / STAGES) & 1);
+      issue_s(sn, j + 1);
+    }
+    float p[32];
+#pragma unroll
+    for (int i = 0; i < 32; ++i) p[i] = sc[i];
+    float mx0 = m0, mx1 = m1;
+#pragma unroll
+    for (int nt = 0; nt < 8; ++nt) {
+      const int key = j * BKV + nt * 8 + 2 * t4;
+#pragma unroll
+      for (int e = 0; e < 2; ++e) {
+        const bool live = key + e < T;
+        p[4 * nt + e] = live ? p[4 * nt + e] * kScale : -INFINITY;
+        p[4 * nt + 2 + e] = live ? p[4 * nt + 2 + e] * kScale : -INFINITY;
+        mx0 = fmaxf(mx0, p[4 * nt + e]); mx1 = fmaxf(mx1, p[4 * nt + 2 + e]);
+      }
+    }
+    mx0 = fmaxf(mx0, __shfl_xor_sync(0xffffffffu, mx0, 1)); mx0 = fmaxf(mx0, __shfl_xor_sync(0xffffffffu, mx0, 2));
+    mx1 = fmaxf(mx1, __shfl_xor_sync(0xffffffffu, mx1, 1)); mx1 = fmaxf(mx1, __shfl_xor_sync(0xffffffffu, mx1, 2));
+    const float alpha0 = ex2(m0 - mx0), alpha1 = ex2(m1 - mx1);
+    m0 = mx0; m1 = mx1;
+    float r0 = 0.f, r1 = 0.f;
+#pragma unroll
+    for (int nt = 0; nt < 8; ++nt) {
+      p[4 * nt + 0] = ex2(p[4 * nt + 0] - mx0); p[4 * nt + 1] = ex2(p[4 * nt + 1] - mx0);
+      p[4 * nt + 2] = ex2(p[4 * nt + 2] - mx1); p[4 * nt + 3] = ex2(p[4 * nt + 3] - mx1);
+      r0 += p[4 * nt + 0] + p[4 * nt + 1]; r1 += p[4 * nt + 2] + p[4 * nt + 3];
+    }
+    l0 = l0 * alpha0 + r0; l1 = l1 * alpha1 + r1;
+
+    uint32_t ph[4][4], pl[4][4];
+#pragma unroll
+    for (int ks = 0; ks < 4; ++ks) {
+#pragma unroll
+      for (int i = 0; i < 4; ++i) {
+        const float a = p[8 * ks + 2 * i], b = p[8 * ks + 2 * i + 1];
+        if constexpr (BF16) ph[ks][i] = pack_bf16x2(a, b);
+        else split_f16x2(a * P_SCALE, b * P_SCALE, ph[ks][i], pl[ks][i]);
+      }
+    }
+    const uint32_t sb = stage_addr(j);
+    const uint64_t dv_hi = make_desc_mn(sb + C::V_OFF), dv_lo = make_desc_mn(sb + C::V_OFF + TILE_BYTES);
+    float pv[32];
+#pragma unroll
+    for (int i = 0; i < 32; ++i) pv[i] = 0.f;
+    fence_regs<32>(pv);
+    wgmma_fence();
+#pragma unroll
+    for (int ks = 0; ks < 4; ++ks) {
+      const uint64_t adv = (uint64_t)((ks * 2048) >> 4);
+      wgmma_m64n64_rs_tb<BF16>(pv, ph[ks], dv_hi + adv, ks != 0 ? 1u : 0u);
+      if constexpr (!BF16) {
+        wgmma_m64n64_rs_tb<false>(pv, pl[ks], dv_hi + adv, 1u);
+        wgmma_m64n64_rs_tb<false>(pv, ph[ks], dv_lo + adv, 1u);
+      }
+    }
+    wgmma_commit();
+    fence_regs<32>(pv);
+    wgmma_wait<0>();
+    fence_regs<32>(pv);
+    fence_regs<32>(sn);
+    if (t == 0) mbar_arrive(smem_u32(empty_bar + j % STAGES));
+#pragma unroll
+    for (int nd = 0; nd < 8; ++nd) {
+      o[4 * nd + 0] = o[4 * nd + 0] * alpha0 + pv[4 * nd + 0]; o[4 * nd + 1] = o[4 * nd + 1] * alpha0 + pv[4 * nd + 1];
+      o[4 * nd + 2] = o[4 * nd + 2] * alpha1 + pv[4 * nd + 2]; o[4 * nd + 3] = o[4 * nd + 3] * alpha1 + pv[4 * nd + 3];
+    }
+  };
+
+  float sa[32], sb[32];
+  mbar_wait(smem_u32(q_bar), 0);
+  mbar_wait(smem_u32(full_bar), 0);
+  issue_s(sa, 0);
+  wgmma_wait<0>();
+  fence_regs<32>(sa);
+  for (int j = 0; j < nblk; j += 2) {
+    block(sa, sb, j);
+    if (j + 1 < nblk) block(sb, sa, j + 1);
+  }
+
+  l0 += __shfl_xor_sync(0xffffffffu, l0, 1); l0 += __shfl_xor_sync(0xffffffffu, l0, 2);
+  l1 += __shfl_xor_sync(0xffffffffu, l1, 1); l1 += __shfl_xor_sync(0xffffffffu, l1, 2);
+  const float inv0 = 1.0f / (l0 * P_SCALE), inv1 = 1.0f / (l1 * P_SCALE);
+  const int q0 = qt * BQ + cw * 64 + warp * 16 + g;
+#pragma unroll
+  for (int half = 0; half < 2; ++half) {
+    const int q = q0 + 8 * half;
+    if (q >= T) continue;
+    const float inv = half ? inv1 : inv0;
+    const size_t off = (out0 + q) * (size_t)D + (size_t)h * HD + 2 * t4;
+#pragma unroll
+    for (int nd = 0; nd < 8; ++nd) {
+      const float a = o[4 * nd + 2 * half] * inv, c = o[4 * nd + 2 * half + 1] * inv;
+      if constexpr (BF16) {
+        *reinterpret_cast<uint32_t*>(reinterpret_cast<__nv_bfloat16*>(o_hi_) + off + nd * 8) = pack_bf16x2(a, c);
+      } else {
+        uint32_t hh, ll;
+        split_f16x2(a, c, hh, ll);
+        *reinterpret_cast<uint32_t*>(reinterpret_cast<__half*>(o_hi_) + off + nd * 8) = hh;
+        *reinterpret_cast<uint32_t*>(reinterpret_cast<__half*>(o_lo_) + off + nd * 8) = ll;
+      }
+    }
+  }
+}
+
+template <bool BF16>
+__global__ void __launch_bounds__(THREADS, 1)
+attention_wg_kernel(const __grid_constant__ CUtensorMap tm_hi, const __grid_constant__ CUtensorMap tm_lo, int T, int D,
+                    void* __restrict__ o_hi, void* __restrict__ o_lo) {
+  attention_wg_cta<BF16, false>(&tm_hi, &tm_lo, T, D, o_hi, o_lo, nullptr);
+}
+
+template <bool BF16>
+__global__ void __launch_bounds__(THREADS, 1)
+attention_wg_varlen_kernel(const __grid_constant__ CUtensorMap tm_hi, const __grid_constant__ CUtensorMap tm_lo,
+                           const __grid_constant__ VarlenAttnTable tab, int D, void* __restrict__ o_hi,
+                           void* __restrict__ o_lo) {
+  attention_wg_cta<BF16, true>(&tm_hi, &tm_lo, 0, D, o_hi, o_lo, &tab);
+}
+
+template <bool BF16>
+static int set_smem_attrs() {
+  static unsigned long long seen = 0;
+  if (first_use_on_this_device(&seen)) {
+    ANYLOC_CHECK_CUDA(cudaFuncSetAttribute(attention_wg_kernel<BF16>, cudaFuncAttributeMaxDynamicSharedMemorySize,
+                                           Cfg<BF16>::SMEM_BYTES));
+    ANYLOC_CHECK_CUDA(cudaFuncSetAttribute(attention_wg_varlen_kernel<BF16>,
+                                           cudaFuncAttributeMaxDynamicSharedMemorySize, Cfg<BF16>::SMEM_BYTES));
+  }
+  return ANYLOC_OK;
+}
+
+}
+
+int attention_wg_launch(const void* qkv_hi, const void* qkv_lo, int B, int T, int D, int heads, void* o_hi, void* o_lo,
+                        bool bf16, cudaStream_t st) {
+  using namespace awg;
+  CUtensorMap m_hi, m_lo;
+  int rc;
+  if ((rc = tc::make_map_3d16(&m_hi, qkv_hi, B, T, 3 * D, 64, bf16))) return rc;
+  if ((rc = tc::make_map_3d16(&m_lo, bf16 ? qkv_hi : qkv_lo, B, T, 3 * D, 64, bf16))) return rc;
+  const dim3 grid(cdiv(T, BQ), heads, B);
+  if (bf16) {
+    if ((rc = set_smem_attrs<true>())) return rc;
+    attention_wg_kernel<true><<<grid, THREADS, Cfg<true>::SMEM_BYTES, st>>>(m_hi, m_lo, T, D, o_hi, o_lo);
+  } else {
+    if ((rc = set_smem_attrs<false>())) return rc;
+    attention_wg_kernel<false><<<grid, THREADS, Cfg<false>::SMEM_BYTES, st>>>(m_hi, m_lo, T, D, o_hi, o_lo);
+  }
+  ANYLOC_CHECK_LAUNCH();
+  return ANYLOC_OK;
+}
+
+int attention_wg_varlen_launch(const void* qkv_hi, const void* qkv_lo, const VarlenAttnTable& tab, int D, int heads,
+                               void* o_hi, void* o_lo, bool bf16, cudaStream_t st) {
+  using namespace awg;
+  VarlenAttnTable t = tab;
+  int tiles = 0, rows = 0;
+  for (int k = 0; k < t.n; ++k) {
+    t.tile0[k] = tiles;
+    tiles += cdiv(t.len[k], BQ);
+    if (t.row0[k] + t.len[k] > rows) rows = t.row0[k] + t.len[k];
+  }
+  CUtensorMap m_hi, m_lo;
+  int rc;
+  if ((rc = tc::make_map_3d16(&m_hi, qkv_hi, 1, rows, 3 * D, 64, bf16))) return rc;
+  if ((rc = tc::make_map_3d16(&m_lo, bf16 ? qkv_hi : qkv_lo, 1, rows, 3 * D, 64, bf16))) return rc;
+  const dim3 grid(tiles, heads);
+  if (bf16) {
+    if ((rc = set_smem_attrs<true>())) return rc;
+    attention_wg_varlen_kernel<true><<<grid, THREADS, Cfg<true>::SMEM_BYTES, st>>>(m_hi, m_lo, t, D, o_hi, o_lo);
+  } else {
+    if ((rc = set_smem_attrs<false>())) return rc;
+    attention_wg_varlen_kernel<false><<<grid, THREADS, Cfg<false>::SMEM_BYTES, st>>>(m_hi, m_lo, t, D, o_hi, o_lo);
+  }
+  ANYLOC_CHECK_LAUNCH();
+  return ANYLOC_OK;
+}
+
+}
diff --git a/anyloc_b200/csrc/gemm_tc.cu b/anyloc_b200/csrc/gemm_tc.cu
--- a/anyloc_b200/csrc/gemm_tc.cu
+++ b/anyloc_b200/csrc/gemm_tc.cu
@@ -441,6 +441,20 @@
   return ANYLOC_OK;
 }
 
+int make_map_3d16(CUtensorMap* map, const void* ptr, int imgs, int rows, int cols, int box_rows, bool bf16) {
+  EncodeTiledFn enc = get_encode();
+  if (!enc) { set_error("tensor map: cuTensorMapEncodeTiled unavailable"); return ANYLOC_ERR_CUDA; }
+  cuuint64_t dims[3] = {(cuuint64_t)cols, (cuuint64_t)rows, (cuuint64_t)imgs};
+  cuuint64_t strides[2] = {(cuuint64_t)cols * 2, (cuuint64_t)rows * cols * 2};
+  cuuint32_t box[3] = {64, (cuuint32_t)box_rows, 1};
+  cuuint32_t estr[3] = {1, 1, 1};
+  CUresult r = enc(map, bf16 ? CU_TENSOR_MAP_DATA_TYPE_BFLOAT16 : CU_TENSOR_MAP_DATA_TYPE_FLOAT16, 3, (void*)ptr, dims,
+                   strides, box, estr, CU_TENSOR_MAP_INTERLEAVE_NONE, CU_TENSOR_MAP_SWIZZLE_128B,
+                   CU_TENSOR_MAP_L2_PROMOTION_L2_256B, CU_TENSOR_MAP_FLOAT_OOB_FILL_NONE);
+  if (r != CUDA_SUCCESS) { set_error("tensor map: cuTensorMapEncodeTiled failed (%d) imgs=%d rows=%d cols=%d", (int)r, imgs, rows, cols); return ANYLOC_ERR_CUDA; }
+  return ANYLOC_OK;
+}
+
 static int make_out_map(CUtensorMap* map, const void* ptr, int rows, int cols, int ld, int esz, int box_cols,
                         bool bf16 = false) {
   EncodeTiledFn enc = get_encode();
diff --git a/anyloc_b200/csrc/tc_common.cuh b/anyloc_b200/csrc/tc_common.cuh
--- a/anyloc_b200/csrc/tc_common.cuh
+++ b/anyloc_b200/csrc/tc_common.cuh
@@ -129,7 +129,63 @@
       : "l"(adesc), "l"(bdesc), "r"(scale_d));
 }
 
+__device__ __forceinline__ void tma_load_3d(uint32_t dst, const CUtensorMap* map, uint32_t bar, int c0, int c1, int c2) {
+  asm volatile(
+      "cp.async.bulk.tensor.3d.shared::cluster.global.mbarrier::complete_tx::bytes [%0], [%1, {%3, %4, %5}], [%2];"
+      ::"r"(dst), "l"(map), "r"(bar), "r"(c0), "r"(c1), "r"(c2) : "memory");
+}
+
+template <int N> __device__ __forceinline__ void setmaxnreg_dec() { asm volatile("setmaxnreg.dec.sync.aligned.u32 %0;" ::"n"(N)); }
+template <int N> __device__ __forceinline__ void setmaxnreg_inc() { asm volatile("setmaxnreg.inc.sync.aligned.u32 %0;" ::"n"(N)); }
+
+__device__ __forceinline__ uint64_t make_desc_mn(uint32_t saddr) {
+  uint64_t d = 0;
+  d |= (uint64_t)((saddr & 0x3FFFF) >> 4);
+  d |= (uint64_t)(1024 >> 4) << 16;
+  d |= (uint64_t)(1024 >> 4) << 32;
+  d |= (uint64_t)1 << 62;
+  return d;
+}
+
+#define ANYLOC_WG_D32                                                                                               \
+  "+f"(d[0]), "+f"(d[1]), "+f"(d[2]), "+f"(d[3]), "+f"(d[4]), "+f"(d[5]), "+f"(d[6]), "+f"(d[7]), "+f"(d[8]),       \
+      "+f"(d[9]), "+f"(d[10]), "+f"(d[11]), "+f"(d[12]), "+f"(d[13]), "+f"(d[14]), "+f"(d[15]), "+f"(d[16]),        \
+      "+f"(d[17]), "+f"(d[18]), "+f"(d[19]), "+f"(d[20]), "+f"(d[21]), "+f"(d[22]), "+f"(d[23]), "+f"(d[24]),       \
+      "+f"(d[25]), "+f"(d[26]), "+f"(d[27]), "+f"(d[28]), "+f"(d[29]), "+f"(d[30]), "+f"(d[31])
+#define ANYLOC_WG_D32_STR                                                                                           \
+  "{%0, %1, %2, %3, %4, %5, %6, %7, %8, %9, %10, %11, %12, %13, %14, %15, %16, %17, %18, %19, %20, %21, %22, %23, " \
+  "%24, %25, %26, %27, %28, %29, %30, %31}"
+
+template <bool BF16>
+__device__ __forceinline__ void wgmma_m64n64_ss(float* d, uint64_t adesc, uint64_t bdesc, uint32_t scale_d) {
+  if constexpr (BF16)
+    asm volatile("{\n\t.reg .pred p;\n\tsetp.ne.b32 p, %34, 0;\n\t"
+                 "wgmma.mma_async.sync.aligned.m64n64k16.f32.bf16.bf16 " ANYLOC_WG_D32_STR ", %32, %33, p, 1, 1, 0, 0;\n\t}"
+                 : ANYLOC_WG_D32 : "l"(adesc), "l"(bdesc), "r"(scale_d));
+  else
+    asm volatile("{\n\t.reg .pred p;\n\tsetp.ne.b32 p, %34, 0;\n\t"
+                 "wgmma.mma_async.sync.aligned.m64n64k16.f32.f16.f16 " ANYLOC_WG_D32_STR ", %32, %33, p, 1, 1, 0, 0;\n\t}"
+                 : ANYLOC_WG_D32 : "l"(adesc), "l"(bdesc), "r"(scale_d));
+}
+
+template <bool BF16>
+__device__ __forceinline__ void wgmma_m64n64_rs_tb(float* d, const uint32_t* a, uint64_t bdesc, uint32_t scale_d) {
+  if constexpr (BF16)
+    asm volatile("{\n\t.reg .pred p;\n\tsetp.ne.b32 p, %37, 0;\n\t"
+                 "wgmma.mma_async.sync.aligned.m64n64k16.f32.bf16.bf16 " ANYLOC_WG_D32_STR
+                 ", {%32, %33, %34, %35}, %36, p, 1, 1, 1;\n\t}"
+                 : ANYLOC_WG_D32 : "r"(a[0]), "r"(a[1]), "r"(a[2]), "r"(a[3]), "l"(bdesc), "r"(scale_d));
+  else
+    asm volatile("{\n\t.reg .pred p;\n\tsetp.ne.b32 p, %37, 0;\n\t"
+                 "wgmma.mma_async.sync.aligned.m64n64k16.f32.f16.f16 " ANYLOC_WG_D32_STR
+                 ", {%32, %33, %34, %35}, %36, p, 1, 1, 1;\n\t}"
+                 : ANYLOC_WG_D32 : "r"(a[0]), "r"(a[1]), "r"(a[2]), "r"(a[3]), "l"(bdesc), "r"(scale_d));
+}
+#undef ANYLOC_WG_D32
+#undef ANYLOC_WG_D32_STR
+
 int make_map(CUtensorMap* map, const void* ptr, int rows, int K, int ld, int box_rows, bool f16, bool bf16 = false);
+int make_map_3d16(CUtensorMap* map, const void* ptr, int imgs, int rows, int cols, int box_rows, bool bf16);
 
 }
 }
```

Result: faster. 180.6, median of 6 (+5.8%).
